# jaeyoungchoilab/Topsicle

Measured on AMD Instinct MI355X. Metric: bases_scanned_per_sec, higher is better.
Workload: dtype u8

## Files before the change

### __graft_entry__.py

```python
import os
import shutil
import subprocess
import sys

ROOT = os.path.dirname(os.path.abspath(__file__))
CSRC = os.path.join(ROOT, "topsicle_amd", "csrc")
LIB = os.path.join(ROOT, "topsicle_amd", "libtopsicle_hip.so")


def _newer(target, deps):
    return os.path.exists(target) and all(os.path.getmtime(target) >= os.path.getmtime(d) for d in deps)


HIP_FLAGS = ["--offload-arch=gfx950", "-O3", "-fno-vectorize", "-std=c++17", "-fPIC", "-Wall", "-Wno-unused-variable"]
KGROUPS = 18


def _build_hip_split(out, extra=()):
    hipcc = shutil.which("hipcc") or "/opt/rocm/bin/hipcc"
    flags = os.environ.get("TPS_HIPCC_EXTRA", "").split() + HIP_FLAGS + list(extra)
    bdir = os.path.join(CSRC, "_build", os.path.splitext(os.path.basename(out))[0])
    os.makedirs(bdir, exist_ok=True)
    jobs = []
    for g in range(KGROUPS):
        src = "topsicle_hip.hip" if g == 0 else "tps_kernels.hip"
        obj = os.path.join(bdir, f"group{g}.o")
        jobs.append((obj, subprocess.Popen([hipcc] + flags + [f"-DTPS_KGROUP={g}", "-c", "-o", obj, os.path.join(CSRC, src)], cwd=CSRC)))
    failed = [obj for obj, p in jobs if p.wait() != 0]
    if failed:
        raise RuntimeError("hipcc failed for " + ", ".join(failed))
    subprocess.check_call([hipcc, "--offload-arch=gfx950", "-shared", "-fPIC", "-o", out] + [obj for obj, _ in jobs], cwd=CSRC)
    return out


def build_hip(force=False):
    deps = [os.path.join(CSRC, f) for f in ("topsicle_hip.hip", "tps_kernels.hip", "tps_kernels.h", "tps_device.h", "tps_wave.h", "tps_plan.h", "tps_pack.h", "tps_wide.h", "tps_wide_plan.h", "tps_motif.h", "tps_variant.h", "tps_tract.h", "tps_ends.h", "tps_anchor.h", "tps_place.h", "tps_adapter.h", "tps_check.h", "tps_layout.h")] + \
           [os.path.join(ROOT, "include", "topsicle_hip.h")]
    if not force and _newer(LIB, deps):
        return LIB
    return _build_hip_split(LIB)


def build_hip_diag():
    return _build_hip_split(os.path.join(ROOT, "topsicle_amd", "libtopsicle_hip_diag.so"), extra=["-DTPS_STAMPS"])


def build_io(force=False):
    src = os.path.join(CSRC, "tps_io.cpp")
    out = os.path.join(ROOT, "topsicle_amd", "libtopsicle_io.so")
    if not force and _newer(out, [src, os.path.join(CSRC, "tps_pack.h"), os.path.join(CSRC, "tps_gzpar.h"), os.path.join(ROOT, "include", "topsicle_hip.h")]):
        return out
    subprocess.check_call(["g++", "-O2", "-std=c++17", "-shared", "-fPIC", "-Wall", "-o", out, src, "-lz", "-lpthread"])
    return out


def build_oracle():
    mk = os.path.join(ROOT, "oracle", "Makefile")
    if os.path.exists(mk):
        subprocess.check_call(["make", "-s", "-C", os.path.join(ROOT, "oracle")])


def build_emulation():
    sys.path.insert(0, os.path.join(ROOT, "tests"))
    sys.path.insert(0, ROOT)
    import emu_adapter_driver
    import emu_anchor_driver
    import emu_binseg_driver
    import emu_clear_driver
    import emu_driver
    import emu_ends_driver
    import emu_follow_wide_driver
    import emu_motif_driver
    import emu_place_driver
    import emu_tract_driver
    import emu_variant_driver
    import emu_wide_driver
    emu_driver.build()
    emu_binseg_driver.build()
    emu_wide_driver.build()
    emu_wide_driver.build_main()
    emu_follow_wide_driver.build()
    emu_motif_driver.build()
    emu_motif_driver.build_main()
    emu_variant_driver.build()
    emu_variant_driver.build_main()
    emu_tract_driver.build()
    emu_tract_driver.build_main()
    emu_ends_driver.build()
    emu_ends_driver.build_main()
    emu_anchor_driver.build()
    emu_anchor_driver.build_main()
    emu_place_driver.build()
    emu_place_driver.build_main()
    emu_adapter_driver.build()
    emu_adapter_driver.build_main()
    emu_clear_driver.build_main()
    import test_layout
    test_layout.build_main()


def build_sanitizer_variants():
    sys.path.insert(0, os.path.join(ROOT, "tests"))
    sys.path.insert(0, ROOT)
    import emu_driver
    import emu_follow_wide_driver
    import emu_wide_driver
    import test_sanitizers
    emu_driver.build(asan=True)
    emu_wide_driver.build(asan=True)
    emu_follow_wide_driver.build(asan=True)
    test_sanitizers._build_io_asan()


def build() -> None:
    import threading
    errs = []

    def side(fn):
        try:
            fn()
        except BaseException as e:
            errs.append(e)
    th = [threading.Thread(target=side, args=(fn,)) for fn in (build_emulation, build_sanitizer_variants)]
    for t in th:
        t.start()
    build_hip()
    build_io()
    build_oracle()
    for t in th:
        t.join()
    if errs:
        raise errs[0]
    sys.path.insert(0, ROOT)
    import topsicle_amd
    from topsicle_amd import hiplib
    lib = hiplib.load_library()
    assert lib.tps_abi_version() == 4
    print("built", LIB)


def _revcomp(s):
    return s[::-1].translate(str.maketrans("ACGT", "TGCA"))


def smoke() -> None:
    sys.path.insert(0, ROOT)
    sys.path.insert(0, os.path.join(ROOT, "oracle"))
    import numpy as np
    from topsicle_amd import hiplib, synth
    import topsicle_oracle as orc

    motif, k = "CCCTAA", 4
    pats = orc.kmer_table(motif, k)
    bases, offsets, _ = synth.make_reads(24, 3000, motif, seed=7, tract_min=300, tract_max=1500)
    seqs = synth.split_reads(bases, offsets)
    ratio = 1000 / len(motif)
    min_count = max(c for c in range(1001) if not (c / ratio > 0.4))
    with hiplib.HipScanner(0) as sc:
        print("smoke on:", sc.device_info())
        sc.set_patterns(pats)
        sc.upload(0, bases, offsets)
        prm = hiplib.make_params(min_len=1000, min_count=min_count, window=100, slide=6, trimfirst=100, maxlen=20000,
                                 flags=hiplib.F_STEP1 | hiplib.F_WINDOWS | hiplib.F_BINSEG | hiplib.F_STORE_SUMS)
        sc.scan(0, prm)
        sc.sync()
        res = sc.results(0)
        sums, win_off = sc.window_sums(0)
        sk, kept = sc.end_sketch(0, motif, res["tail"] != 0, [1500] * len(seqs), [3500] * len(seqs))
        degree, links, matches = sc.sketch_links(np.vstack([sk, sk]), 6, 4)
        assert (kept > 200).all() and (links[:len(seqs), 0] == np.arange(len(seqs)) + len(seqs)).all() and (matches[:len(seqs), 0] == (sk != 0xFFFFFFFF).sum(axis=1)).all()
        codes, keep = sc.end_window(0, motif, res["tail"] != 0, [1500] * len(seqs), [3500] * len(seqs))
        n_keep = np.array([sum(bin(int(x)).count("1") for x in row) for row in keep])
        offset, votes, second = sc.anchor_offsets(codes, keep, [1500] * len(seqs), list(range(len(seqs))), 2000)
        assert (n_keep == kept).all() and (offset == 0).all() and (2 * votes > kept).all() and (votes <= kept).all() and (4 * second < votes).all()
        p_ref, p_total, _, _, p_offset, p_votes, _ = sc.place_windows(codes, keep, [1500] * len(seqs), codes[:5], keep[:5], [1500] * 5, 2000)
        assert (p_ref[:5] == np.arange(5)).all() and (p_total[:5] >= kept[:5]).all() and (p_offset[:5] == 0).all() and (2 * p_votes[:5] > kept[:5]).all() and (p_votes[5:] < 20).all()
        ad = ["GATTACAGGCATCGTTCAGAGTCC", "TGCATCAGGTCCAAGTCAGGTTCA"]
        planted = seqs[0][:7] + ad[0][:11] + ad[0][12:] + seqs[0][30:] if res["tail"][0] == 0 else seqs[0][:-30] + _revcomp(ad[0][:11] + ad[0][12:]) + seqs[0][-7:]
        sc.upload(1, *hiplib.pack_reads([planted] + seqs[1:]))
        a_dist, a_end = sc.adapter_find(1, ad, res["tail"] != 0, [0] * len(seqs), [256] * len(seqs))
        assert (int(a_dist[0, 0]), int(a_end[0, 0])) == (1, 30) and (a_dist[1:, 0] > 5).all() and (a_dist[:, 1] > 5).all() and (a_end <= 256).all()
# ... 22 lines not shown
```

### include/topsicle_hip.h

```cpp
#ifndef TOPSICLE_HIP_H
#define TOPSICLE_HIP_H

#include <stdint.h>

#ifdef __cplusplus
extern "C" {
#endif

#define TPS_ABI_VERSION 4

#define TPS_OK            0
#define TPS_E_NO_DEVICE  -1
#define TPS_E_HIP        -2
#define TPS_E_ARG        -3
#define TPS_E_PATTERN    -4
#define TPS_E_CAPACITY   -5
#define TPS_E_STATE      -6

#define TPS_MAX_K         15
#define TPS_DIRECT_K      7
#define TPS_MAX_PATTERNS 31
#define TPS_WIDE_MAX_K        32
#define TPS_WIDE_MAX_PATTERNS 64

// ... 71 lines not shown
                               int64_t n_reads, int64_t n_words, int64_t* n_words_out);
int  tps_batch_set_tails(tps_ctx* ctx, int32_t slot, const uint8_t* tails);

int  tps_batch_scan(tps_ctx* ctx, int32_t slot, const tps_params* prm);
int  tps_sync(tps_ctx* ctx);
int  tps_batch_results(tps_ctx* ctx, int32_t slot, tps_read_result* out, int64_t n_reads);
int  tps_batch_window_offsets(tps_ctx* ctx, int32_t slot, int64_t* win_off, int64_t n_plus_1);
int  tps_batch_window_sums(tps_ctx* ctx, int32_t slot, int32_t* sums, int64_t n_windows);
int  tps_batch_window_raw(tps_ctx* ctx, int32_t slot, uint8_t* raw, int64_t n_windows_times_p);
typedef uint32_t (*tps_crc32_fn)(uint32_t crc, const uint8_t* p, int64_t n);
int  tps_batch_raw_to_fd(tps_ctx* ctx, int32_t slot, const int64_t* reads, int64_t n_sel, int fd, int64_t file_off,
                         tps_crc32_fn crc_fn, uint32_t* crc_out, int64_t* bytes_out);
int  tps_batch_read_sums(tps_ctx* ctx, int32_t slot, int64_t read, int32_t* sums, int64_t n_windows);
int  tps_batch_trc_counts(tps_ctx* ctx, int32_t slot, int32_t* c_start, int32_t* c_end, int64_t n_reads);

int  tps_trc_counts(tps_ctx* ctx, const uint8_t* bases, const int64_t* offsets, int64_t n_reads,
                    int32_t no_bp, int32_t* c_start, int32_t* c_end);
int  tps_window_counts(tps_ctx* ctx, const uint8_t* bases, const int64_t* offsets,
                       const uint8_t* tails, int64_t n_reads, int32_t window, int32_t slide,
                       int32_t trimfirst, int32_t maxlen, const int64_t* win_off,
                       int32_t* sums, uint8_t* raw);
int  tps_binseg_l2(tps_ctx* ctx, const int32_t* sums, const int64_t* win_off, int64_t n_reads,
                   int32_t n_patterns, int32_t jump, int32_t min_size, int32_t* bkp, double* gain);
int  tps_binseg_l2_ties(tps_ctx* ctx, const int32_t* sums, const int64_t* win_off, int64_t n_reads,
                        int32_t n_patterns, int32_t jump, int32_t min_size, int32_t* bkp, double* gain, uint8_t* tie);

int64_t tps_window_count(int64_t read_len, int32_t window, int32_t slide, int32_t trimfirst, int32_t maxlen);

int  tps_batch_kmer_followers(tps_ctx* ctx, int32_t slot, int32_t n_fwd, int32_t follow, int32_t lo, int32_t hi,
                              int32_t min_len, uint32_t* picks, int64_t picks_words, int64_t* hist, int64_t hist_len);
int  tps_batch_kmer_followers_wide(tps_ctx* ctx, int32_t slot, int32_t n_fwd, int32_t follow, int32_t lo, int32_t hi,
                                   int32_t min_len, uint32_t* picks, int64_t picks_words, int64_t* hist, int64_t hist_len);

typedef struct tps_motif_hit {
    uint64_t unit;
    int32_t period;
    int32_t support;
    int32_t run_start;
    int32_t run_len;
    int32_t n_bases;
    int32_t reserved;
} tps_motif_hit;
int  tps_batch_motif_census(tps_ctx* ctx, int32_t slot, int32_t u_min, int32_t u_max, int32_t lo, int32_t hi, int32_t min_len,
                            tps_motif_hit* hits, int64_t n_hits, int32_t* counts, int64_t counts_len);

int  tps_batch_variant_census(tps_ctx* ctx, int32_t slot, uint64_t unit, int32_t m, const uint8_t* tails, const int32_t* begin,
                              const int32_t* end, int64_t n_reads, int32_t bin, int32_t n_bins, uint32_t* counts,
                              int64_t counts_len, int64_t* profile, int64_t profile_len);

typedef struct tps_tract {
    int32_t begin, end;
    int32_t hits, blocks;
} tps_tract;
int  tps_batch_tract_map(tps_ctx* ctx, int32_t slot, uint64_t unit, int32_t m, int32_t block, int32_t min_hits, int32_t gap,
                         int32_t min_blocks, int32_t max_tracts, tps_tract* tracts, int64_t tracts_len, int32_t* found,
                         int64_t found_len, uint32_t* totals, int64_t totals_len);

int  tps_batch_end_sketch(tps_ctx* ctx, int32_t slot, uint64_t unit, int32_t m, int32_t k, int32_t buckets, const uint8_t* tails,
                          const int32_t* begin, const int32_t* end, int64_t n_reads, uint32_t* sketch, int64_t sketch_len,
                          uint32_t* kept, int64_t kept_len);
int  tps_sketch_links(tps_ctx* ctx, const uint32_t* sketch, int64_t n, int32_t buckets, int64_t sketch_len, int32_t min_match,
                      int32_t max_links, int32_t* degree, int64_t degree_len, int32_t* links, int64_t links_len, int32_t* matches,
                      int64_t matches_len);

int  tps_batch_end_window(tps_ctx* ctx, int32_t slot, uint64_t unit, int32_t m, int32_t k, const uint8_t* tails, const int32_t* begin,
                          const int32_t* end, int64_t n_reads, int32_t span, uint32_t* codes, int64_t codes_len, uint32_t* keep,
                          int64_t keep_len);
int  tps_window_offsets(tps_ctx* ctx, const uint32_t* codes, const uint32_t* keep, const int32_t* length, const int32_t* ref, int64_t n,
                        int32_t span, int32_t k, int32_t* offset, int32_t* votes, int32_t* second, int64_t out_len);

int  tps_window_place(tps_ctx* ctx, const uint32_t* codes, int64_t codes_len, const uint32_t* keep, int64_t keep_len, const int32_t* length,
                      int64_t n, const uint32_t* ref_codes, int64_t ref_codes_len, const uint32_t* ref_keep, int64_t ref_keep_len,
                      const int32_t* ref_length, int32_t n_ref, int32_t span, int32_t k, int32_t max_occ, int32_t* ref, int32_t* total,
                      int32_t* runner_ref, int32_t* runner, int32_t* offset, int32_t* votes, int32_t* second, int64_t out_len);

int  tps_batch_adapter_find(tps_ctx* ctx, int32_t slot, const uint64_t* patterns, const int32_t* pat_len, int32_t n_pat,
                            const uint8_t* tails, const int32_t* begin, const int32_t* end, int64_t n_reads, uint16_t* hits,
                            int64_t hits_len);

int  tps_kernel_time_ms(tps_ctx* ctx, int32_t* n_launches, double* total_ms, double* mean_ms);
int  tps_kernel_time_reset(tps_ctx* ctx);
int  tps_ctx_debug_option(tps_ctx* ctx, const char* key, int64_t value);
int  tps_debug_stamps_get(tps_ctx* ctx, int32_t slot, uint64_t* out, int64_t n_reads);
int  tps_device_info(tps_ctx* ctx, char* buf, int32_t buf_len);
int  tps_batch_kernel_info(tps_ctx* ctx, int32_t slot, char* buf, int32_t buf_len);

#ifdef __cplusplus
}
#endif
#endif
```

### topsicle_amd/csrc/topsicle_hip.hip

```cpp
#include <hip/hip_runtime.h>
#include <hip/hip_ext.h>

#include <sys/uio.h>
#include <unistd.h>

#include <algorithm>
#include <cerrno>
#include <cstdarg>
#include <cstdio>
#include <cstdlib>
#include <cstring>
#include <deque>
#include <initializer_list>
#include <map>
#include <mutex>
#include <set>
#include <string>
#include <vector>

#include "tps_device.h"
#include "tps_motif.h"
#include "tps_variant.h"
#include "tps_tract.h"
#include "tps_ends.h"
// ... 204 lines not shown
            uint64_t x;
            if (!rev) {
                x = nib_swap(q[w]);
            } else {
                const int64_t a = L - 16 - 16 * w;
                const int64_t qa = a >> 4;
                const uint32_t sh = (uint32_t)(a & 15) * 4u;
                const uint64_t lo = qa >= 0 ? nib_swap(q[qa]) : 0ull;
                x = sh ? (lo >> sh) | (nib_swap(q[qa + 1]) << (64u - sh)) : lo;
                x = __brevll(x);
            }
#pragma unroll
            for (int t = 0; t < 16; ++t) {
                const uint32_t c = (uint32_t)(x >> (4 * t)) & 15u;
                packed |= ((NIB4_CODE2 >> (2 * c)) & 3u) << (2 * t);
                bad |= ((~NIB4_ACGT >> c) & 1u) << t;
            }
            if (left < 16) {
                packed &= (1u << (2 * (int)left)) - 1u;
                bad &= (1u << (int)left) - 1u;
            }
        }
        seq2[w0 + w] = packed;
        inv[w0 + w] = (uint16_t)bad;
    }
}

namespace {

thread_local std::string g_err;

std::mutex g_pinned_mu;
std::map<uintptr_t, size_t> g_pinned;
bool is_pinned(const void* p, size_t bytes) {
    if (!p || !bytes) return true;
    std::lock_guard<std::mutex> lk(g_pinned_mu);
    auto it = g_pinned.upper_bound((uintptr_t)p);
    if (it == g_pinned.begin()) return false;
    --it;
    return (uintptr_t)p + bytes <= it->first + it->second;
}

int fail(int code, const char* fmt, ...) {
    char buf[512];
    va_list ap;
    va_start(ap, fmt);
    vsnprintf(buf, sizeof buf, fmt, ap);
    va_end(ap);
    g_err = buf;
    return code;
}

#define HIP_TRY(expr)                                                                        \
    do {                                                                                     \
        hipError_t e_ = (expr);                                                              \
        if (e_ != hipSuccess) return fail(TPS_E_HIP, "%s: %s", #expr, hipGetErrorString(e_)); \
    } while (0)

constexpr int64_t PAD = 64;
constexpr int INTERNAL_SLOT = TPS_MAX_SLOTS;

struct DevBuf {
    void* p = nullptr;
    size_t cap = 0;
    bool borrowed = false;
    DevBuf() = default;
    DevBuf(const DevBuf&) = delete;
    DevBuf& operator=(const DevBuf&) = delete;
    ~DevBuf() { release(); }
    int ensure(size_t bytes) {
        if (borrowed) { p = nullptr; cap = 0; borrowed = false; }
        if (bytes <= cap) return TPS_OK;
        if (p) { (void)hipFree(p); p = nullptr; cap = 0; }
        size_t want = bytes + bytes / 8 + 256;
        HIP_TRY(hipMalloc(&p, want));
        cap = want;
        return TPS_OK;
    }
    void release() { if (p && !borrowed) (void)hipFree(p); p = nullptr; cap = 0; borrowed = false; }
    void borrow(const DevBuf& o) { release(); p = o.p; cap = o.cap; borrowed = true; }
};

struct Slot {
    DevBuf seq2, inv, desc, tails, results, c_start, c_end, win_off, win_off16, sums, raw, stamps, lc, order;
    int64_t n_words = 0;
    bool inv_valid = true;
    bool any_invalid = true;
    std::vector<int64_t> h_offsets;
    tps::BatchLayout lay;
    std::vector<uint16_t> h_sums16;
    tps_read_result* h_results = nullptr;
    size_t h_results_cap = 0;
    int64_t n = -1;
    bool has_tails = false;
    bool planned = false;
    tps_params plan_prm{};
    int plan_k = 0, plan_p = 0;
    uint32_t plan_dup = 0, plan_so = 0;
    tps::ScanArgs args{};
    size_t lds_bytes = 0;
    const char* kernel_name = "";
    bool scanned = false;
    uint32_t last_flags = 0;
    Slot* sub = nullptr;
    bool sub_stale = true;
    void* ext_raw = nullptr;
    const int64_t* ext_raw_win_off = nullptr;
    bool rows_inline = false;
    int stride_base = 0;
    std::string info_name;
    bool wplanned = false;
    tps_params wplan_prm{};
    uint64_t wplan_table = 0;
    tps::WideArgs wargs{};
    ~Slot() {
        if (h_results) (void)hipHostFree(h_results);
        delete sub;
    }
};

struct ScanKernel { const void* fn; const char* name; };
#define TPS_K(sym) {(const void*)sym, #sym}
enum ScanFamily { KF_PLAIN, KF_PAIR, KF_PAIRQ, KF_RAW, KF_SO, KF_SOL, KF_SOR, KF_SORH, KF_COUNT };
constexpr int KSLIDE_MIN = 3, KSLIDE_MAX = 12;
const ScanKernel GENERIC_KERNEL = TPS_K(tps_scan_kernel);
const ScanKernel FUSED_KERNELS[KF_COUNT][KSLIDE_MAX - KSLIDE_MIN + 1] = {
    {TPS_K(tps_scan_kernel_s3), TPS_K(tps_scan_kernel_s4), TPS_K(tps_scan_kernel_s5), TPS_K(tps_scan_kernel_s6), TPS_K(tps_scan_kernel_s7),
     TPS_K(tps_scan_kernel_s8), TPS_K(tps_scan_kernel_s9), TPS_K(tps_scan_kernel_s10), TPS_K(tps_scan_kernel_s11), TPS_K(tps_scan_kernel_s12)},
    {TPS_K(tps_scan_kernel_s3p), TPS_K(tps_scan_kernel_s4p), TPS_K(tps_scan_kernel_s5p), TPS_K(tps_scan_kernel_s6p), TPS_K(tps_scan_kernel_s7p),
     TPS_K(tps_scan_kernel_s8p), TPS_K(tps_scan_kernel_s9p), TPS_K(tps_scan_kernel_s10p), TPS_K(tps_scan_kernel_s11p), TPS_K(tps_scan_kernel_s12p)},
    {{}, {}, TPS_K(tps_scan_kernel_s5q), TPS_K(tps_scan_kernel_s6q), TPS_K(tps_scan_kernel_s7q), TPS_K(tps_scan_kernel_s8q)},
    {{}, {}, TPS_K(tps_scan_kernel_s5r), TPS_K(tps_scan_kernel_s6r), TPS_K(tps_scan_kernel_s7r), TPS_K(tps_scan_kernel_s8r)},
    {{}, {}, TPS_K(tps_scan_kernel_s5so), TPS_K(tps_scan_kernel_s6so), TPS_K(tps_scan_kernel_s7so), TPS_K(tps_scan_kernel_s8so)},
    {{}, {}, TPS_K(tps_scan_kernel_s5sol), TPS_K(tps_scan_kernel_s6sol), TPS_K(tps_scan_kernel_s7sol), TPS_K(tps_scan_kernel_s8sol)},
    {{}, {}, TPS_K(tps_scan_kernel_s5sor), TPS_K(tps_scan_kernel_s6sor), TPS_K(tps_scan_kernel_s7sor), TPS_K(tps_scan_kernel_s8sor)},
    {{}, {}, TPS_K(tps_scan_kernel_s5sorh), TPS_K(tps_scan_kernel_s6sorh), TPS_K(tps_scan_kernel_s7sorh), TPS_K(tps_scan_kernel_s8sorh)},
};
#undef TPS_K

struct EventPair { hipEvent_t a, b; };

}

struct tps_ctx {
    int device = 0;
    hipStream_t stream = nullptr;
    hipDeviceProp_t prop{};
    struct Table { DevBuf dev; int P = 0, k = 0; std::string key; tps::PatInfo pat{}; size_t off_e32 = 0, off_fld = 0, off_m16 = 0, off_f16 = 0, off_p16 = 0, off_pfld = 0; };
    std::deque<Table> tables;
    Table* lut_cur = nullptr;
    struct WideTable { DevBuf dev; std::string key; int P = 0, k = 0; tps::WidePat pat{}; uint64_t serial = 0; };
    std::deque<WideTable> wtables;
    WideTable* wide_cur = nullptr;
    size_t wtable_rr = 0;
    uint64_t table_serial = 0;
    size_t lds_set_wide = 0;
    size_t table_rr = 0;
    DevBuf follow_picks, follow_hist;
    DevBuf motif_hits, motif_counts;
    DevBuf variant_in, variant_counts, variant_prof;
    std::vector<unsigned long long> h_variant_prof;
    DevBuf tract_table, tract_out;
    DevBuf ends_in, ends_out;
    DevBuf links_t, links_out;
    DevBuf window_out;
    DevBuf offsets_in, offsets_out;
    DevBuf place_in, place_idx, place_out;
    DevBuf adapter_in, adapter_out;
    DevBuf ascii, ascii_off;
    DevBuf nib, nib_src;
    std::set<void*> pinned;
    std::vector<tps_read_desc> h_desc;
    tps::PatInfo pat{};
// ... 335 lines not shown
        sl.wplan_table = wt.serial;
        sl.wplanned = true;
    }
    sl.planned = false;
    sl.args = tps::ScanArgs{};
    sl.args.wpg = sl.wargs.wpg;
    sl.plan_p = P;
    sl.plan_k = wt.k;
    sl.stride_base = 0;
    sl.rows_inline = false;
    sl.lds_bytes = (size_t)tps::wide_wg_lds_dwords(sl.wargs) * 4;
    static const char wide_name[] = "tps_scan_kernel_wide";
    sl.kernel_name = wide_name;
    sl.last_flags = prm.flags;
    const int64_t total_win = sl.lay.win_off[(size_t)n];
    if ((rc = ensure_h_results(sl, n))) return rc;
    tps::WideArgs& a = sl.wargs;
    a.seq2 = (const uint32_t*)sl.seq2.p;
    a.inv = (const uint16_t*)sl.inv.p;
    a.desc = (const tps_read_desc*)sl.desc.p;
    a.tails_in = ((prm.flags & TPS_F_TAILS_IN) && !(prm.flags & TPS_F_STEP1)) ? (const uint8_t*)sl.tails.p : nullptr;
    a.img = (const uint32_t*)wt.dev.p;
    a.results = sl.h_results;
    a.c_start = a.c_end = nullptr;
    if (prm.flags & TPS_F_STEP1) {
        if ((rc = sl.c_start.ensure((size_t)std::max<int64_t>(n * P, 1) * 4))) return rc;
        if ((rc = sl.c_end.ensure((size_t)std::max<int64_t>(n * P, 1) * 4))) return rc;
        a.c_start = (int32_t*)sl.c_start.p;
        a.c_end = (int32_t*)sl.c_end.p;
    }
    a.win_off = (const int64_t*)sl.win_off.p;
    a.order = sl.lay.order.empty() ? nullptr : (const int32_t*)sl.order.p;
    a.sums = nullptr;
    a.raw = nullptr;
    if (prm.flags & TPS_F_WINDOWS) {
        if ((rc = sl.sums.ensure((size_t)std::max<int64_t>(total_win, 1) * 4))) return rc;
        a.sums = (int32_t*)sl.sums.p;
    }
    if (prm.flags & TPS_F_STORE_RAW) {
        if ((rc = sl.raw.ensure((size_t)std::max<int64_t>(total_win * P, 1)))) return rc;
        a.raw = (uint8_t*)sl.raw.p;
    }
    a.n_reads = n;
    a.prm = prm;
    if (n == 0) { sl.scanned = true; return TPS_OK; }
    if (c->poison) {
        if ((rc = poison_h_results(c, sl))) return rc;
        if (a.c_start) { TPS_POISON(sl.c_start); TPS_POISON(sl.c_end); }
        if (a.sums) TPS_POISON(sl.sums);
        if (a.raw) TPS_POISON(sl.raw);
    }
    if (sl.lds_bytes > c->lds_set_wide) {
        HIP_TRY(hipFuncSetAttribute((const void*)tps_scan_kernel_wide, hipFuncAttributeMaxDynamicSharedMemorySize, (int)sl.lds_bytes));
        c->lds_set_wide = sl.lds_bytes;
    }
    EventPair ev;
    if ((rc = next_events(c, false, ev))) return rc;
    const int64_t grid = (n + a.wpg - 1) / a.wpg;
    void* kargs[] = {(void*)&a};
    HIP_TRY(hipExtLaunchKernel((const void*)tps_scan_kernel_wide, dim3((unsigned)grid), dim3(tps::NT * a.wpg), kargs, sl.lds_bytes, c->stream,
                               ev.a, ev.b, 0));
    sl.scanned = true;
    return TPS_OK;
}

int do_scan(tps_ctx* c, Slot& sl, const tps_params& prm, bool inner, hipEvent_t ev_start) {
    int rc;
    if (!c->have_pat) return fail(TPS_E_PATTERN, "tps_set_patterns has not been called");
    if ((rc = check_scan(sl, prm))) return rc;
    if (c->wide_cur) return do_scan_wide(c, sl, prm);
    const int64_t n = sl.n;
    const int P = c->pat.P;
    if (!sl.planned || !same_params(prm, sl.plan_prm) || sl.plan_k != c->pat.k || sl.plan_p != P ||
        (sl.plan_dup != 0) != (c->pat.dup_mask != 0) || (sl.plan_so != 0) != (c->pat.so_mask != 0)) {
        tps::plan_batch_layout(sl.h_offsets.data(), n, prm, sl.lay);
        if (c->file_order) sl.lay.order.clear();
        if (!sl.lay.order.empty()) {
            if ((rc = sl.order.ensure((size_t)n * 4))) return rc;
            HIP_TRY(hipMemcpyAsync(sl.order.p, sl.lay.order.data(), (size_t)n * 4, hipMemcpyHostToDevice, c->stream));
        }
        sl.args = tps::ScanArgs{};
        sl.args.val_on = sl.any_invalid ? 1 : 0;
        if ((rc = plan_lds(c, sl, prm, sl.lay.max_nwin))) return rc;
        sl.stride_base = 0;
        if (!inner && !c->no_stride) {
            sl.stride_base = tps::stride_base(sl.args, prm, c->pat.k, P, [&](int s0) { return window_count(sl.lay.max_len, prm.window, s0, prm.trimfirst, prm.maxlen); },
                                              lds_budget_dw(c), c->knobs);
        }
        if ((rc = sl.win_off.ensure((size_t)(n + 1) * 8))) return rc;
        HIP_TRY(hipMemcpyAsync(sl.win_off.p, sl.lay.win_off.data(), (size_t)(n + 1) * 8, hipMemcpyHostToDevice, c->stream));
        if (sl.args.variant) {
            if ((rc = sl.win_off16.ensure((size_t)(n + 1) * 8))) return rc;
            HIP_TRY(hipMemcpyAsync(sl.win_off16.p, sl.lay.win_off16.data(), (size_t)(n + 1) * 8, hipMemcpyHostToDevice, c->stream));
        }
        HIP_TRY(hipStreamSynchronize(c->stream));
        sl.plan_prm = prm;
        sl.plan_k = c->pat.k;
        sl.plan_p = P;
        sl.plan_dup = c->pat.dup_mask;
        sl.plan_so = c->pat.so_mask;
        sl.planned = true;
    }
    const int64_t total_win = sl.lay.win_off[(size_t)n];
    if ((rc = ensure_h_results(sl, n))) return rc;
    tps::ScanArgs& a = sl.args;
    a.seq2 = (const uint32_t*)sl.seq2.p;
    a.inv = (const uint16_t*)sl.inv.p;
    a.desc = (const tps_read_desc*)sl.desc.p;
    a.tails_in = ((prm.flags & TPS_F_TAILS_IN) && !(prm.flags & TPS_F_STEP1)) ? (const uint8_t*)sl.tails.p : nullptr;
    a.lut = (const uint32_t*)c->lut_cur->dev.p;
    a.pair_img = a.lut + (a.pair16 ? c->lut_cur->off_p16 : (a.lut_fields && a.pair_n) ? c->lut_cur->off_pfld : (size_t)a.lut_n);
    a.lut_img = a.lut + ((a.lut16 && a.lut_fields) ? c->lut_cur->off_f16 : a.lut16 ? c->lut_cur->off_m16 : a.lut_fields ? c->lut_cur->off_fld : c->lut_cur->off_e32);
    a.results = sl.h_results;
    if (inner) {
        if ((rc = sl.results.ensure((size_t)std::max<int64_t>(n, 1) * sizeof(tps_read_result)))) return rc;
        a.results = (tps_read_result*)sl.results.p;
    }
    a.c_start = a.c_end = nullptr;
    if ((prm.flags & TPS_F_STEP1) && !sl.stride_base) {
        if ((rc = sl.c_start.ensure((size_t)std::max<int64_t>(n * P, 1) * 4))) return rc;
        if ((rc = sl.c_end.ensure((size_t)std::max<int64_t>(n * P, 1) * 4))) return rc;
        a.c_start = (int32_t*)sl.c_start.p;
        a.c_end = (int32_t*)sl.c_end.p;
    }
    a.win_off = (const int64_t*)sl.win_off.p;
    a.order = sl.lay.order.empty() ? nullptr : (const int32_t*)sl.order.p;
    a.sums = nullptr;
    a.sums16 = nullptr;
    a.win_off16 = nullptr;
    a.raw = nullptr;
    if (prm.flags & TPS_F_WINDOWS) {
        if (a.variant) {
            if ((rc = sl.sums.ensure((size_t)std::max<int64_t>(sl.lay.win_off16[(size_t)n], 8) * 2))) return rc;
            a.sums16 = (uint16_t*)sl.sums.p;
            a.win_off16 = (const int64_t*)sl.win_off16.p;
        } else {
            if ((rc = sl.sums.ensure((size_t)std::max<int64_t>(total_win, 1) * 4))) return rc;
            a.sums = (int32_t*)sl.sums.p;
        }
    }
    a.raw_m = 0;
    a.raw_win_off = nullptr;
    sl.rows_inline = false;
    if (prm.flags & TPS_F_STORE_RAW) {
        if (inner && sl.ext_raw && a.variant && a.pp_d >= 0 && (c->pat.so_mask == 0 ? a.pp_d == 0 : a.pp_d > 0) && (P & 3) == 0 && !sl.any_invalid) {
            a.raw = (uint8_t*)sl.ext_raw;
            a.raw_m = 2;
            a.raw_win_off = sl.ext_raw_win_off;
            sl.rows_inline = true;
        } else {
            if ((rc = sl.raw.ensure((size_t)std::max<int64_t>(total_win * P, 1)))) return rc;
            a.raw = (uint8_t*)sl.raw.p;
        }
    }
    a.lc_scratch = nullptr;
    if (a.lc_global) {
        if ((rc = sl.lc.ensure((size_t)std::max<int64_t>(n, 1) * (size_t)a.lc_stride * 2))) return rc;
        a.lc_scratch = (uint16_t*)sl.lc.p;
    }
    if (c->poison) {
        if (inner) TPS_POISON(sl.results);
        else if ((rc = poison_h_results(c, sl))) return rc;
        if (a.c_start) { TPS_POISON(sl.c_start); TPS_POISON(sl.c_end); }
        if (a.sums || a.sums16) TPS_POISON(sl.sums);
        if (a.raw && !sl.rows_inline) TPS_POISON(sl.raw);
        if (a.lc_scratch) TPS_POISON(sl.lc);
    }
    a.stamps = nullptr;
    if (c->want_stamps) {
        if ((rc = sl.stamps.ensure((size_t)std::max<int64_t>(n, 1) * 16 * 8))) return rc;
        TPS_POISON(sl.stamps);
        HIP_TRY(hipMemsetAsync(sl.stamps.p, 0, (size_t)std::max<int64_t>(n, 1) * 16 * 8, c->stream));
        a.stamps = (uint64_t*)sl.stamps.p;
    }
    a.n_reads = n;
    a.pat = c->pat;
    a.prm = prm;
    sl.last_flags = prm.flags;
    if (n == 0) { sl.scanned = true; return TPS_OK; }

    const ScanKernel* k = &GENERIC_KERNEL;
    size_t* lds_set = &c->lds_set_generic;
    if (tps::has_specialised_slide(a.variant) || tps::has_default_only_slide(a.variant)) {
        const ScanFamily fam = scan_family(a, a.raw != nullptr);
        k = &FUSED_KERNELS[fam][a.variant - KSLIDE_MIN];
        lds_set = &c->lds_set_fused[fam][a.variant - KSLIDE_MIN];
    }
    sl.kernel_name = k->name;
    if (sl.lds_bytes > *lds_set) {
        HIP_TRY(hipFuncSetAttribute(k->fn, hipFuncAttributeMaxDynamicSharedMemorySize, (int)sl.lds_bytes));
        *lds_set = sl.lds_bytes;
    }
    EventPair ev;
    if ((rc = next_events(c, inner, ev))) return rc;
    if (sl.stride_base) {
        if ((rc = do_scan_strided(c, sl, prm, sl.stride_base, ev.a, ev.b))) return rc;
        sl.scanned = true;
        return TPS_OK;
    }
    {
        const int64_t grid = (n + a.wpg - 1) / a.wpg;
        void* kargs[] = {(void*)&a};
        HIP_TRY(hipExtLaunchKernel(k->fn, dim3((unsigned)grid), dim3(tps::NT * a.wpg), kargs, sl.lds_bytes, c->stream,
                                   inner ? ev_start : ev.a, ev.b, 0));
    }
    sl.scanned = true;
    return TPS_OK;
}

Slot* get_slot(tps_ctx* c, int slot) {
    if (!c || slot < 0 || slot >= TPS_MAX_SLOTS) { fail(TPS_E_ARG, "slot out of range"); return nullptr; }
    return &c->slots[slot];
}


int need_slot(tps_ctx* c, int slot, Slot** out) {
    int rc;
    if ((rc = bind(c))) return rc;
    return (*out = get_slot(c, slot)) ? TPS_OK : TPS_E_ARG;
}
int have_batch(const Slot& sl) { return sl.n < 0 ? fail(TPS_E_STATE, "no batch uploaded in this slot") : TPS_OK; }
int need_batch(tps_ctx* c, int slot, Slot** out) {
    int rc;
    if ((rc = need_slot(c, slot, out))) return rc;
    return have_batch(**out);
}

template <class A>
void set_batch(A& a, const Slot& sl) {
    a.seq2 = (const uint32_t*)sl.seq2.p;
    a.inv = (const uint16_t*)sl.inv.p;
    a.desc = (const tps_read_desc*)sl.desc.p;
}

template <class T>
T* at(const DevBuf& b, size_t off) { return (T*)((char*)b.p + off); }

template <class A>
int upload_region(tps_ctx* c, const DevBuf& buf, const tps::RegionAt& r, const uint8_t* tails, const int32_t* begin, const int32_t* end, int64_t n, A& a) {
    a.tails = at<const uint8_t>(buf, r.tails);
    a.begin = at<const int32_t>(buf, r.begin);
    a.end = at<const int32_t>(buf, r.end);
    HIP_TRY(hipMemcpyAsync((void*)a.tails, tails, (size_t)n, hipMemcpyHostToDevice, c->stream));
    HIP_TRY(hipMemcpyAsync((void*)a.begin, begin, (size_t)n * 4, hipMemcpyHostToDevice, c->stream));
    HIP_TRY(hipMemcpyAsync((void*)a.end, end, (size_t)n * 4, hipMemcpyHostToDevice, c->stream));
    return TPS_OK;
}
// ... 654 lines not shown
    const tps::RegionAt reg = tps::region_layout(in, n);
    if ((rc = c->adapter_in.ensure(in.total))) return rc;
    if ((rc = c->adapter_out.ensure(out_bytes))) return rc;
    TPS_POISON(c->adapter_out);
    tps::AdapterArgs a{};
    set_batch(a, *sl);
    a.peq = at<const uint64_t>(c->adapter_in, off_peq);
    a.pat_len = at<const int32_t>(c->adapter_in, off_len);
    HIP_TRY(hipMemcpyAsync((void*)a.peq, peq, peq_bytes, hipMemcpyHostToDevice, c->stream));
    HIP_TRY(hipMemcpyAsync((void*)a.pat_len, pat_len, len_bytes, hipMemcpyHostToDevice, c->stream));
    if ((rc = upload_region(c, c->adapter_in, reg, tails, begin, end, n, a))) return rc;
    a.hits = (uint32_t*)c->adapter_out.p;
    a.n_reads = n;
    a.n_pat = n_pat;
    if ((rc = launch_waves(c, tps::adapter_find_kernel, n, tps::ADAPTER_WPG, a))) return rc;
    return download(c, {{hits, a.hits, out_bytes}});
}

int tps_batch_set_tails(tps_ctx* c, int32_t slot, const uint8_t* tails) {
    int rc;
    if ((rc = bind(c))) return rc;
    Slot* sl = get_slot(c, slot);
    if (!sl) return TPS_E_ARG;
    if (sl->n < 0) return fail(TPS_E_STATE, "no batch uploaded in this slot");
    if (!tails && sl->n > 0) return fail(TPS_E_ARG, "null tails");
    if ((rc = sl->tails.ensure((size_t)std::max<int64_t>(sl->n, 1)))) return rc;
    if (sl->n) HIP_TRY(hipMemcpyAsync(sl->tails.p, tails, (size_t)sl->n, hipMemcpyHostToDevice, c->stream));
    HIP_TRY(hipStreamSynchronize(c->stream));
    sl->has_tails = true;
    return TPS_OK;
}

int tps_batch_scan(tps_ctx* c, int32_t slot, const tps_params* prm) {
    int rc;
    if ((rc = bind(c))) return rc;
    Slot* sl = get_slot(c, slot);
    if (!sl) return TPS_E_ARG;
    if (!prm) return fail(TPS_E_ARG, "null params");
    return do_scan(c, *sl, *prm);
}

int tps_sync(tps_ctx* c) {
    int rc;
    if ((rc = bind(c))) return rc;
    HIP_TRY(hipStreamSynchronize(c->stream));
    return TPS_OK;
}

static int need_scanned(tps_ctx* c, int slot, Slot** out) {
    int rc;
    if ((rc = bind(c))) return rc;
    Slot* sl = (slot == INTERNAL_SLOT) ? &c->slots[INTERNAL_SLOT] : get_slot(c, slot);
    if (!sl) return TPS_E_ARG;
    if (!sl->scanned) return fail(TPS_E_STATE, "slot has not been scanned");
    HIP_TRY(hipStreamSynchronize(c->stream));
    *out = sl;
    return TPS_OK;
}

int tps_batch_results(tps_ctx* c, int32_t slot, tps_read_result* out, int64_t n) {
    Slot* sl;
    int rc;
    if ((rc = need_scanned(c, slot, &sl))) return rc;
    if (n != sl->n || (n > 0 && !out)) return fail(TPS_E_ARG, "result buffer must hold %lld reads", (long long)sl->n);
    if (n) memcpy(out, sl->h_results, (size_t)n * sizeof(tps_read_result));
    return TPS_OK;
}

int tps_batch_window_offsets(tps_ctx* c, int32_t slot, int64_t* win_off, int64_t n1) {
    Slot* sl;
    int rc;
    if ((rc = need_scanned(c, slot, &sl))) return rc;
    if (n1 != sl->n + 1 || !win_off) return fail(TPS_E_ARG, "win_off must hold n+1 entries");
    memcpy(win_off, sl->lay.win_off.data(), (size_t)n1 * 8);
    return TPS_OK;
}

int tps_batch_window_sums(tps_ctx* c, int32_t slot, int32_t* sums, int64_t nw) {
    Slot* sl;
    int rc;
    if ((rc = need_scanned(c, slot, &sl))) return rc;
    if (!(sl->last_flags & TPS_F_STORE_SUMS)) return fail(TPS_E_STATE, "last scan did not store window sums");
    if (nw != sl->lay.win_off[(size_t)sl->n] || (nw > 0 && !sums)) return fail(TPS_E_ARG, "sums must hold %lld windows", (long long)sl->lay.win_off[(size_t)sl->n]);
    if (nw && sl->args.variant) {
        const int64_t n16 = sl->lay.win_off16[(size_t)sl->n];
        sl->h_sums16.resize((size_t)n16);
        HIP_TRY(hipMemcpy(sl->h_sums16.data(), sl->sums.p, (size_t)n16 * 2, hipMemcpyDeviceToHost));
        tps::widen_sums16(sl->h_sums16.data(), sl->lay.win_off16.data(), sl->lay.win_off.data(), 0, sl->n, sums);
    } else if (nw) {
        HIP_TRY(hipMemcpy(sums, sl->sums.p, (size_t)nw * 4, hipMemcpyDeviceToHost));
    }
    tps::clear_skipped_windows(sl->h_results, sl->lay.win_off.data(), sl->n, 1, 4, 0, nw, sums);
    return TPS_OK;
}

int tps_batch_read_sums(tps_ctx* c, int32_t slot, int64_t read, int32_t* sums, int64_t nw) {
    Slot* sl;
    int rc;
    if ((rc = need_scanned(c, slot, &sl))) return rc;
    if (!(sl->last_flags & TPS_F_WINDOWS)) return fail(TPS_E_STATE, "last scan did not run the window step");
    if (read < 0 || read >= sl->n) return fail(TPS_E_ARG, "read %lld out of range", (long long)read);
    const int64_t lo = sl->lay.win_off[(size_t)read], cnt = sl->lay.win_off[(size_t)read + 1] - lo;
    if (nw != cnt || (nw > 0 && !sums)) return fail(TPS_E_ARG, "sums must hold %lld windows", (long long)cnt);
    if (!nw) return TPS_OK;
    if (sl->args.variant) {
        sl->h_sums16.resize((size_t)nw);
        HIP_TRY(hipMemcpy(sl->h_sums16.data(), (const uint16_t*)sl->sums.p + sl->lay.win_off16[(size_t)read], (size_t)nw * 2, hipMemcpyDeviceToHost));
        for (int64_t w = 0; w < nw; ++w) sums[w] = (int32_t)sl->h_sums16[(size_t)w];
    } else {
        HIP_TRY(hipMemcpy(sums, (const int32_t*)sl->sums.p + lo, (size_t)nw * 4, hipMemcpyDeviceToHost));
    }
    tps::clear_skipped_windows(sl->h_results, sl->lay.win_off.data(), sl->n, 1, 4, lo, lo + nw, sums);
    return TPS_OK;
}

int tps_batch_window_raw(tps_ctx* c, int32_t slot, uint8_t* raw, int64_t nwp) {
    Slot* sl;
    int rc;
    if ((rc = need_scanned(c, slot, &sl))) return rc;
    if (!(sl->last_flags & TPS_F_STORE_RAW)) return fail(TPS_E_STATE, "last scan did not store raw counts");
    int64_t want = sl->lay.win_off[(size_t)sl->n] * sl->plan_p;
    if (nwp != want || (nwp > 0 && !raw)) return fail(TPS_E_ARG, "raw must hold %lld bytes", (long long)want);
    if (nwp) HIP_TRY(hipMemcpy(raw, sl->raw.p, (size_t)nwp, hipMemcpyDeviceToHost));
    tps::clear_skipped_windows(sl->h_results, sl->lay.win_off.data(), sl->n, sl->plan_p, 1, 0, nwp, raw);
    return TPS_OK;
}

constexpr size_t RAW_STAGE = (size_t)32 << 20;
constexpr int64_t RAW_GAP = 256 << 10;

int tps_batch_raw_to_fd(tps_ctx* c, int32_t slot, const int64_t* reads, int64_t n_sel, int fd, int64_t file_off,
                        tps_crc32_fn crc_fn, uint32_t* crc_out, int64_t* bytes_out) {
    Slot* sl;
    int rc;
    if ((rc = need_scanned(c, slot, &sl))) return rc;
    if (!(sl->last_flags & TPS_F_STORE_RAW)) return fail(TPS_E_STATE, "last scan did not store raw counts");
    if (n_sel < 0 || (n_sel > 0 && !reads) || fd < 0 || file_off < 0) return fail(TPS_E_ARG, "bad arguments");
    if (crc_out) *crc_out = 0;
    if (bytes_out) *bytes_out = 0;
    const int64_t P = sl->plan_p;
    struct Run { int64_t lo, hi; };
    std::vector<Run> runs;
    int64_t prev = -1;
    for (int64_t j = 0; j < n_sel; ++j) {
        const int64_t i = reads[j];
        if (i <= prev || i >= sl->n) return fail(TPS_E_ARG, "reads[] must be ascending indices of the batch (entry %lld)", (long long)j);
        prev = i;
        const int64_t lo = sl->lay.win_off[(size_t)i] * P, hi = sl->lay.win_off[(size_t)i + 1] * P;
        if (hi == lo) continue;
        if (!runs.empty() && runs.back().hi == lo) runs.back().hi = hi;
        else runs.push_back({lo, hi});
    }
    if (runs.empty()) return TPS_OK;
    for (int i = 0; i < 2; ++i) {
        if (!c->raw_stage[i]) HIP_TRY(hipHostMalloc(&c->raw_stage[i], RAW_STAGE, hipHostMallocPortable));
        if (!c->raw_ev[i]) HIP_TRY(hipEventCreateWithFlags(&c->raw_ev[i], hipEventDisableTiming));
    }
    struct Piece { size_t r0, r1; int64_t lo, hi; };
    std::vector<Piece> pieces;
    {
        std::vector<Run> cut;
        size_t i = 0;
        int64_t pos = runs[0].lo;
        while (i < runs.size()) {
            Piece pc{cut.size(), cut.size(), pos, pos};
            while (i < runs.size()) {
                const int64_t start = std::max(pos, runs[i].lo);
                if (pc.r1 > pc.r0 && (start - pc.hi > RAW_GAP || start >= pc.lo + (int64_t)RAW_STAGE)) break;
                if (pc.r1 == pc.r0) pc.lo = start;
                const int64_t end = std::min(runs[i].hi, pc.lo + (int64_t)RAW_STAGE);
                if (end <= start) break;
                cut.push_back({start, end});
                pc.r1 = cut.size();
                pc.hi = end;
                pos = end;
                if (end == runs[i].hi) { ++i; if (i < runs.size()) pos = runs[i].lo; }
                else break;
            }
            pieces.push_back(pc);
        }
        runs.swap(cut);
    }
    auto enqueue = [&](size_t j) -> int {
        const Piece& pc = pieces[j];
        HIP_TRY(hipMemcpyAsync(c->raw_stage[j & 1], (const uint8_t*)sl->raw.p + pc.lo, (size_t)(pc.hi - pc.lo), hipMemcpyDeviceToHost, c->stream));
        HIP_TRY(hipEventRecord(c->raw_ev[j & 1], c->stream));
        return TPS_OK;
    };
// ... 105 lines not shown
    if (nw > 0 && !sums) return fail(TPS_E_ARG, "null sums");
    for (int64_t i = 0; i < n; ++i) {
        const int64_t lo = win_off[i], len = win_off[i + 1] - lo;
        if (len < 0 || lo < 0 || lo + len > nw) return fail(TPS_E_ARG, "win_off not monotone at %lld", (long long)i);
        if (len > 500000) return fail(TPS_E_CAPACITY, "read %lld has %lld windows (max 500000)", (long long)i, (long long)len);
        uint64_t tot = 0;
        for (int64_t w = 0; w < len; ++w) {
            if (sums[lo + w] < 0) return fail(TPS_E_ARG, "negative window sum at read %lld", (long long)i);
            tot += (uint64_t)sums[lo + w];
        }
        if (tot >> 32 || (double)len * (double)len * (double)tot >= 18446744073709551616.0)
            return fail(TPS_E_CAPACITY, "window sums of read %lld exceed the change-point arithmetic (total %llu over %lld windows)",
                        (long long)i, (unsigned long long)tot, (long long)len);
    }
    Slot& sl = c->slots[INTERNAL_SLOT];
    if ((rc = sl.sums.ensure((size_t)std::max<int64_t>(nw, 1) * 4))) return rc;
    if ((rc = sl.win_off.ensure((size_t)(n + 1) * 8))) return rc;
    if ((rc = sl.results.ensure((size_t)n * 17))) return rc;
    TPS_POISON(sl.results);
    sl.planned = false;
    sl.wplanned = false;
    sl.scanned = false;
    if (nw) HIP_TRY(hipMemcpyAsync(sl.sums.p, sums, (size_t)nw * 4, hipMemcpyHostToDevice, c->stream));
    HIP_TRY(hipMemcpyAsync(sl.win_off.p, win_off, (size_t)(n + 1) * 8, hipMemcpyHostToDevice, c->stream));
    tps::BinsegArgs a{};
    a.sums = (const int32_t*)sl.sums.p;
    a.win_off = (const int64_t*)sl.win_off.p;
    a.gain = (double*)sl.results.p;
    a.bkp = (int32_t*)((char*)sl.results.p + (size_t)n * 8);
    a.tie = (uint8_t*)sl.results.p + (size_t)n * 12;
    a.n_reads = n;
    a.n_patterns = n_patterns;
    a.jump = jump;
    a.min_size = min_size;
    hipLaunchKernelGGL(tps_binseg_kernel, dim3((unsigned)((n + tps::WPG - 1) / tps::WPG)), dim3(tps::NT * tps::WPG), 0, c->stream, a);
    HIP_TRY(hipGetLastError());
    HIP_TRY(hipMemcpyAsync(bkp, a.bkp, (size_t)n * 4, hipMemcpyDeviceToHost, c->stream));
    if (gain) HIP_TRY(hipMemcpyAsync(gain, a.gain, (size_t)n * 8, hipMemcpyDeviceToHost, c->stream));
    if (tie) HIP_TRY(hipMemcpyAsync(tie, a.tie, (size_t)n, hipMemcpyDeviceToHost, c->stream));
    HIP_TRY(hipStreamSynchronize(c->stream));
    return TPS_OK;
}

int tps_kernel_time_ms(tps_ctx* c, int32_t* n_launches, double* total_ms, double* mean_ms) {
    int rc;
    if ((rc = bind(c))) return rc;
    HIP_TRY(hipStreamSynchronize(c->stream));
    double tot = 0.0;
    for (size_t i = c->ev_base; i < c->ev_used; ++i) {
        float ms = 0.f;
        HIP_TRY(hipEventElapsedTime(&ms, c->ev_pool[i].a, c->ev_pool[i].b));
        tot += ms;
    }
    const size_t cnt = c->ev_used - c->ev_base;
    if (n_launches) *n_launches = (int32_t)cnt;
    if (total_ms) *total_ms = tot;
    if (mean_ms) *mean_ms = cnt ? tot / (double)cnt : 0.0;
    return TPS_OK;
}

int tps_ctx_debug_option(tps_ctx* c, const char* key, int64_t value) {
    if (!c || !key) return fail(TPS_E_ARG, "null argument");
    const std::string k(key);
    if (k == "event_stride") c->event_stride = (int)std::max<int64_t>(1, value);
    else if (k == "no_events") c->no_events = value != 0;
    else if (k == "force_generic") c->knobs.force_generic = value != 0;
    else if (k == "spans_per_tile") c->knobs.spans_per_tile = (int)std::max<int64_t>(0, value);
    else if (k == "force_pair") c->knobs.force_pair = value != 0;
    else if (k == "so_order") c->knobs.so_order = (int)value;
    else if (k == "wpg") c->knobs.wpg = (int)value;
    else if (k == "stamps") c->want_stamps = value != 0;
    else if (k == "file_order") c->file_order = value != 0;
    else if (k == "no_stride") c->no_stride = value != 0;
    else if (k == "no_inline_rows") c->no_inline_rows = value != 0;
    else if (k == "poison") {
        if (value < 0 || value > 255) return fail(TPS_E_ARG, "poison must be 0 (off) or a fill byte 1..255");
        c->poison = (int)value;
    }
    else return fail(TPS_E_ARG, "unknown debug option '%s' (event_stride, no_events, force_generic, spans_per_tile, force_pair, so_order, wpg, stamps, file_order, no_stride, no_inline_rows, poison)", key);
    drop_plans(c);
    return TPS_OK;
}

int tps_debug_stamps_get(tps_ctx* c, int32_t slot, uint64_t* out, int64_t n) {
    Slot* sl;
    int rc;
    if ((rc = need_scanned(c, slot, &sl))) return rc;
    if (!sl->stamps.p || n != sl->n) return fail(TPS_E_STATE, "no stamps recorded");
    HIP_TRY(hipMemcpy(out, sl->stamps.p, (size_t)n * 16 * 8, hipMemcpyDeviceToHost));
    return TPS_OK;
}

int tps_kernel_time_reset(tps_ctx* c) {
    int rc;
    if ((rc = bind(c))) return rc;
    HIP_TRY(hipStreamSynchronize(c->stream));
    c->ev_base = c->ev_used;
    c->launch_seq = 0;
    return TPS_OK;
}

}
```

### topsicle_amd/csrc/tps_device.h

```cpp
#pragma once
#include <stdint.h>
#include "../../include/topsicle_hip.h"
#include "tps_wave.h"
#include "tps_check.h"

namespace tps {

constexpr int WPG = 4;
constexpr int WPG_MAX = 8;
constexpr uint32_t FLAG_CONFLICT = 0x80000000u;
constexpr uint32_t FLAG16 = 0x8000u;
constexpr int HIST_COPIES = 8;
constexpr int WIN_U = 4;
constexpr int COOP_MAX = 24;

typedef unsigned __int128 u128;

constexpr int cgcd(int a, int b) { return b == 0 ? a : cgcd(b, a % b); }
constexpr int clog2(int x) { return x <= 1 ? 0 : 1 + clog2(x / 2); }

struct PatInfo {
    int32_t P, k;
    uint32_t kmask;
    uint32_t all_mask;
    uint32_t so_mask;
    uint32_t dup_mask;
    int32_t n_periods;
    int32_t period[8];
    uint32_t period_pat[8];
    uint32_t hash_mul, hash_shift;
};

struct ScanArgs {
    const uint32_t* seq2;
    const uint16_t* inv;
    const tps_read_desc* desc;
    const uint8_t* tails_in;
    const uint32_t* lut;
    const uint32_t* lut_img;
    const uint32_t* pair_img;
    tps_read_result* results;
    int32_t* c_start;
    int32_t* c_end;
    const int64_t* win_off;
    int32_t* sums;
    uint16_t* sums16;
    const int64_t* win_off16;
    uint8_t* raw;
    uint64_t* stamps;
    int32_t raw_m;
    const int64_t* raw_win_off;
    const int32_t* order;
    int64_t n_reads;
    PatInfo pat;
    tps_params prm;
    int32_t variant;
    int32_t lut_n;
    int32_t seq_dw;
    int32_t head_dw;
    int32_t nblk_cap;
    int32_t spans_per_tile;
    int32_t span_dw;
    int32_t blk_log2;
    int32_t rec_rs;
    int32_t tot_dw;
    int32_t blk_dw;
    int32_t lc_cap;
    uint32_t jump_magic;
    int32_t q, r, lw;
    int32_t lc_global;
    int32_t lc_stride;
    uint16_t* lc_scratch;
    int32_t pair_n;
    int32_t tw;
    int32_t tile_full;
    int32_t wpg;
    int32_t pp_d;
    int32_t so_fast;
    int32_t val_on;
    int32_t seq_alias;
    int32_t lut_fields;
    int32_t lut16;
    int32_t xt_alias;
    int32_t xt_own;
    int32_t pair16;
};

struct BinsegArgs {
    const int32_t* sums;
    const int64_t* win_off;
    int32_t* bkp;
    double* gain;
    int64_t n_reads;
    int32_t n_patterns, jump, min_size;
    uint8_t* tie;
};

constexpr int MISC_DW = 20;
constexpr int XS_DW = 64 + NT + 4 * NT + NT + 16 * 5 + 8;
constexpr int HIST_STRIDE = 33;
constexpr int HIST_DW = 2 * HIST_COPIES * HIST_STRIDE;
struct Lds {
    uint32_t* lut;
    uint32_t* lut2;
    int lshift;
    uint32_t* seq2;
    uint16_t* val;
    uint32_t* blk;
    uint32_t* G;
    uint32_t* Gp;
    uint16_t* C0;
    uint16_t* C1;
    uint32_t* XPC;
    uint32_t* XF;
    uint32_t* XT;
    uint32_t* Tot;
    uint32_t* row;
    uint32_t* misc;
};
constexpr int XLANES = NT + 16;
TPS_HD int64_t xchg_dw(const ScanArgs& a) {
    return 9ll * NT + (a.xt_alias == 2 ? 0ll : 2ll) * XLANES;
}
TPS_HD int64_t lut_dw(const ScanArgs& a) { return a.lut16 ? ((((int64_t)a.lut_n + 1) / 2 + 3) & ~3ll) : (((int64_t)a.lut_n + 3) & ~3ll); }
TPS_HD int64_t blk_region_dw(const ScanArgs& a) {
    int64_t need = a.variant ? xchg_dw(a) : 2ll * a.nblk_cap + 2ll * ((a.nblk_cap + 1) / 2);
    if (need < XS_DW) need = XS_DW;
    if (need < HIST_DW) need = HIST_DW;
    return (need + 3) & ~3ll;
}
TPS_HD int64_t val_dw(const ScanArgs& a) { return a.val_on ? ((a.seq_dw + 4 + 3) / 4) * 2 : 0; }
TPS_HD int64_t row_dw(const ScanArgs& a) {
    const int64_t fused = a.variant ? ((int64_t)NT << a.blk_log2) + NT : 0;
    return fused > WIN_U * NT ? fused : WIN_U * NT;
}
TPS_DEV Lds carve(uint32_t* base, uint32_t* lut, const ScanArgs& a) {
    Lds l;
    l.lut2 = lut - a.pair_n;
    uint32_t* p = base;
    l.blk = p;  p += a.blk_dw;
    l.lut = lut;
    l.lshift = a.variant ? 16 : 0;
    l.seq2 = p; p += a.seq_dw;
    l.val = (uint16_t*)p;  p += val_dw(a);
    l.Tot = p;  p += a.tot_dw;
    l.row = p;  p += row_dw(a);
    l.misc = p;
    l.G = l.blk;
    l.Gp = l.G + a.nblk_cap;
    l.C0 = (uint16_t*)(l.Gp + a.nblk_cap);
    l.C1 = l.C0 + ((a.nblk_cap + 1) / 2) * 2;
    l.XPC = l.blk;
    l.XF = l.XPC + 9 * NT;
    l.XT = l.XF + XLANES;
    return l;
}
TPS_HD int64_t lds_dwords(const ScanArgs& a) {
    return (int64_t)a.blk_dw + (a.seq_alias ? 0 : a.seq_dw) + val_dw(a) + a.tot_dw + row_dw(a) + MISC_DW +
           ((a.xt_alias && a.xt_own) ? (a.xt_alias == 2 ? 2 : 1) * XLANES : 0);
}
TPS_HD int64_t wg_lds_dwords(const ScanArgs& a) { return a.pair_n + lut_dw(a) + (int64_t)(a.wpg > 0 ? a.wpg : WPG) * ((lds_dwords(a) + 3) & ~3ll); }
constexpr int M_BEST = 0;
constexpr int M_CMASK = 2;
constexpr int M_INVALID = 4;
constexpr int M_SCAN = 10;
constexpr int M_MAXSC = 6;
constexpr int M_BESTB = 8;
constexpr int M_NTIE = 9;
// ... 666 lines not shown
            scan_positions(l, pat, q0, a.lw, inv, [&](int p, uint32_t h) {
                if ((h >> bit) & 1u) {
                    ++occ;
                    if (p >= cursor) { ++greedy; cursor = p + pat.k; }
                }
            });
            sum -= (uint32_t)(occ - greedy);
        }
        return sum;
    }
    uint64_t clo = 0, chi = 0, c3 = 0, c4 = 0;
    scan_positions(l, pat, q0, a.lw, inv, [&](int, uint32_t h) {
        while (h) {
            const int b = ffs0(h);
            h &= h - 1;
            const uint64_t inc = 1ull << (8 * (b & 7));
            const int g = b >> 3;
            clo += g == 0 ? inc : 0ull;
            chi += g == 1 ? inc : 0ull;
            c3 += g == 2 ? inc : 0ull;
            c4 += g == 3 ? inc : 0ull;
        }
    });
    uint32_t sum = 0;
    for (int b = 0; b < pat.P; ++b) {
        const uint64_t word = (b >> 3) == 0 ? clo : (b >> 3) == 1 ? chi : (b >> 3) == 2 ? c3 : c4;
        int c = (int)((word >> (8 * (b & 7))) & 255u);
        if ((redo >> b) & 1u) {
            int greedy = 0, cursor = 0;
            scan_positions(l, pat, q0, a.lw, inv, [&](int p, uint32_t h) {
                if (((h >> b) & 1u) && p >= cursor) { ++greedy; cursor = p + pat.k; }
            });
            c = greedy;
        }
        if (c == 0) c = 1;
        if (raw_row) raw_row[b] = (uint8_t)c;
        sum += (uint32_t)c;
    }
    return sum;
}

TPS_DEV void windows_group(const ScanArgs& a, const Lds& l, int delta, int w0, int nw_tile, int64_t out_base, int base, int tid) {
    const PatInfo& pat = a.pat;
    const int q = a.q;
    for (int u = 0; u < WIN_U; ++u) {
        const int wl = base + u * NT + tid;
        uint32_t sw = 0;
        if (wl < nw_tile) {
            uint32_t m = l.Gp[wl + q];
            for (int i = 0; i < q; ++i) m |= l.G[wl + i];
            int je = wl + q;
            uint32_t cnt = ((uint32_t)l.C1[je] + l.Tot[je >> a.blk_log2]) - ((uint32_t)l.C0[wl] + l.Tot[wl >> a.blk_log2]);
            uint32_t present = m & pat.all_mask;
            sw = cnt + (uint32_t)(pat.P - popc(present));
            uint8_t* raw_row = a.raw ? a.raw + (out_base + w0 + wl) * (int64_t)pat.P : nullptr;
            if ((m & FLAG_CONFLICT) || raw_row) sw = window_exact(a, l, delta, wl, present, sw, raw_row);
            a.sums[out_base + w0 + wl] = (int32_t)sw;
        }
        l.row[u * NT + tid] = sw;
    }
}

TPS_DEV uint32_t div_jump(uint32_t w, uint32_t magic) { return magic ? (uint32_t)(((uint64_t)w * magic) >> 32) : w; }
TPS_DEV void candidates_group(const ScanArgs& a, const Lds& l, uint64_t lc_g, int w0, int nw_tile, int base, uint32_t carry, int tid) {
    const uint32_t jump = (uint32_t)a.prm.jump;
    TPS_UNROLL
    for (int u = 0; u < WIN_U; ++u) {
        const int wl = base + u * NT + tid;
        if (wl < nw_tile) {
            const uint32_t w = (uint32_t)(w0 + wl);
            const uint32_t c = div_jump(w, a.jump_magic);
            if (c * jump == w && (int)c < a.lc_cap) {
                g32_store(lc_g, c, carry + l.row[u * NT + tid]);
            }
        }
    }
}

struct TileConst {
    int32_t q, r;
    uint32_t jump, jump_magic, lc_cap;
    uint64_t lc_g;
    uint16_t* sw16;
    int64_t rd;
};
TPS_DEV TileConst tile_const(const ScanArgs& a, int64_t r) {
    TileConst t;
    t.lc_g = (uint64_t)(uintptr_t)(a.lc_scratch + r * (int64_t)a.lc_stride);
    t.sw16 = a.sums16 + (a.win_off16 ? a.win_off16[r] : 0);
    t.rd = r;
    t.q = (int32_t)uniform((uint32_t)a.q); t.r = (int32_t)uniform((uint32_t)a.r);
    t.jump = uniform((uint32_t)a.prm.jump); t.jump_magic = uniform(a.jump_magic);
    t.lc_cap = uniform((uint32_t)a.lc_cap);
    TPS_PIN_S(t.q); TPS_PIN_S(t.r); TPS_PIN_S(t.jump); TPS_PIN_S(t.jump_magic); TPS_PIN_S(t.lc_cap);
    return t;
}

template <int S>
struct Geo {
    static constexpr int B = 8;
    static constexpr int LOG2B = 3;
    static constexpr int C = 8;
    static constexpr int LOG2C = 3;
    static constexpr int POS = B * S;
    static constexpr int WDW = (POS + 13 + 15) / 16;
};
constexpr int SEQ_LEAD = 4;
template <int S, bool FULL>
struct TileGeo {
    static constexpr int LANES = FULL ? NT : NT - 1;
    static constexpr int BASES = LANES * Geo<S>::POS + 13 + 15;
    static constexpr int NQ = (63 + BASES + 63) / 64;
    static constexpr int PF = (NQ + NT - 1) / NT;
    static constexpr int SEQ_TILE = SEQ_LEAD + 4 * NQ + 4;
    static constexpr int SEQ = SEQ_TILE < 144 ? 144 : SEQ_TILE;
};
constexpr bool tile_full_default(int s) { return s >= 1; }

template <int S, bool FULL>
TPS_DEV Lds carve_fused(uint32_t* base, uint32_t* lut, const ScanArgs& a) {
    constexpr int BLK = 9 * NT, ROW = NT * Geo<S>::B + NT, SEQ = TileGeo<S, FULL>::SEQ;
    const int VAL = a.val_on ? ((SEQ + 4 + 3) / 4) * 2 : 0;
    static_assert(BLK % 4 == 0 && ROW % 4 == 0 && MISC_DW % 4 == 0 && SEQ % 4 == 0, "seq2 must be 16-byte aligned");
    static_assert(BLK + ROW - SEQ >= HIST_DW && BLK + ROW - SEQ >= 4 * NT, "step 1 counts in front of the aliased bases");
    Lds l;
    l.lut2 = lut - a.pair_n;
    l.lut = lut;
    l.lshift = (a.lut16 && !a.lut_fields && !a.pair16) ? LUT_M16 : (a.lut_fields && a.lut16) ? LUT_F16 : a.lut_fields ? LUT_FIELDS : 16;
    l.blk = base;
    l.XPC = base;
    l.G = l.Gp = base; l.C0 = l.C1 = (uint16_t*)base;
    l.row = base + BLK;
    l.misc = l.row + ROW;
    l.Tot = l.misc + MISC_DW;
    uint32_t* p = l.Tot + 4;
    if (a.seq_alias) {
        l.seq2 = base + (BLK + ROW - SEQ);
    } else {
        l.seq2 = p;
        p += SEQ;
    }
    l.val = (uint16_t*)p;
    p += VAL;
    l.XF = p;
    l.XT = l.XF + XLANES;
    return l;
}

TPS_DEV uint32_t pack_hi_lo(uint32_t hi_src, uint32_t lo_src) { return perm(hi_src, lo_src, 0x07060100u); }

template <int S, bool SO, bool INV, int RPT, bool RAW>
TPS_DEV void tile_fused_s(const ScanArgs& a, const TileConst& tc, const Lds& l, int delta, int w0, int tile, int nw_tile,
                          int64_t out_base, uint64_t& s_total, int64_t r) {
    constexpr bool RZ = RPT == 0;
    typedef Geo<S> g_;
    constexpr int WDW = g_::WDW, B = g_::B, LOG2B = g_::LOG2B, POS = g_::POS;
    constexpr int RS = NT + NT / B;
    const PatInfo& pat = a.pat;
    const int rp = RPT >= 0 ? RPT : tc.r, q = tc.q;
    const uint32_t amask = pat.kmask << 2;
    TPS_PHASE {
        const int span = tid;
        const int p0 = delta + span * POS;
        const uint32_t sh2 = (uint32_t)((p0 - 1) & 15) * 2u;
        const int d0 = (p0 - 1) >> 4;
        uint32_t w[WDW];
        {
            uint32_t prev = l.seq2[d0];
            TPS_UNROLL
            for (int i = 0; i < WDW; ++i) {
                uint32_t nx = l.seq2[d0 + i + 1];
                w[i] = alignbit(nx, prev, sh2);
// ... 604 lines not shown
        uint32_t* const sw = TPS_AT(sw_);
        uint32_t* const swp = TPS_AT(swp_);
        const uint32_t* const sfx = TPS_AT(sfx_);
        const uint32_t* const c0s = TPS_AT(c0s_);
        const uint32_t* pe = l.XPC + (lane + dl0) * (B + 1) + rot;
        uint32_t ev[B];
        TPS_UNROLL
        for (int j = 0; j < B; ++j) ev[j] = pe[j + ((!ROTZ && j >= brk) ? 1 : 0)];
        uint32_t orw = 0, sumw = TPS_AT(xf_own);
        TPS_NOVEC
        for (int t = 1; t < dl0; ++t) {
            const uint32_t v = xf_at(lane + t);
            orw |= v;
            sumw += v;
        }
        uint32_t orb = orw, sumb = sumw;
        if (!ROTZ) {
            const uint32_t vb = xf_at(lane + dl0);
            orb |= vb;
            sumb += vb;
        }
        const uint32_t am = pat.all_mask << 16;
        orw |= ~am;
        orb |= ~am;
        uint32_t run = 0;
        if constexpr (SWP) {
            if (tid == 0) TPS_EMU_COUNT(3);
            uint32_t lo_lo = 0x05040100u;
            TPS_PIN_S(lo_lo);
            TPS_UNROLL
            for (int j = 0; j < B; j += 2) {
                const uint32_t ep = perm(ev[j + 1], ev[j], lo_lo), cp = perm(c0s[j + 1], c0s[j], lo_lo);
                const uint32_t d = pk_u16_add(pk_u16_sub(ep, cp), sumw);
                const uint32_t p = (uint32_t)popc(~(sfx[j] | ev[j] | orw)) + d;
                swp[j >> 1] = p + ((uint32_t)popc(~(sfx[j + 1] | ev[j + 1] | orw)) << 16);
                sw[j] = swp[j >> 1] & 0xFFFFu;
                sw[j + 1] = swp[j >> 1] >> 16;
                run += sw[j] + sw[j + 1];
            }
        } else {
        TPS_UNROLL
        for (int j = 0; j < B; ++j) {
            const bool far_ = !ROTZ && j >= brk;
            const uint32_t e = ev[j], fo = far_ ? orb : orw, fs = far_ ? sumb : sumw;
            const uint32_t c = (e - c0s[j] + fs) & 0xFFFFu;
            sw[j] = (CD > 0 ? (c & 0xFFu) - (c >> 8) : c) + (uint32_t)popc(~(sfx[j] | e | fo));
            run += sw[j];
        }
        }
        TPS_AT(ltot) = run;
    }
    TPS_ISA_MARK(MK + 3);
    if constexpr (CD > 0) {
        const bool tile_chain = lane_chain != 0;
        if (tile_chain) {
            TPS_EMU_COUNT(5);
            LaneArr<uint32_t, B> pd;
            Lane<uint32_t> dt(0);
            TPS_PHASE {
                const uint32_t* pr = l.row + tid * (B + 1);
                TPS_UNROLL
                for (int j = 0; j < B; ++j) { TPS_AT(dt) += pr[j]; TPS_AT(pd)[j] = TPS_AT(dt); }
            }
            const Lane<uint32_t> dbase = wave_excl_sum(dt);
            TPS_LANES {
                uint32_t run = 0;
                TPS_UNROLL
                for (int j = 0; j < B; ++j) { TPS_AT(sw_)[j] += TPS_AT(dbase) + TPS_AT(pd)[j]; run += TPS_AT(sw_)[j]; }
                TPS_AT(ltot) = run;
            }
        } else {
            TPS_EMU_COUNT(6);
        }
    }
    const Lane<uint32_t> lexc = wave_excl_sum(ltot);
    bool lane_cands = false;
    if constexpr (CD == 0 && !M16) lane_cands = tc.jump >= 4u;
    const uint32_t c_lo = div_jump((uint32_t)w0 + tc.jump - 1u, tc.jump_magic);
    uint32_t c_hi = div_jump((uint32_t)(w0 + nw_tile) + tc.jump - 1u, tc.jump_magic);
    if (c_hi > tc.lc_cap) c_hi = tc.lc_cap;
    TPS_PHASE {
        const int lane = tid;
        const uint32_t* const sw = TPS_AT(sw_);
        if constexpr (SWP) g_store_sw8p(tc.sw16 + w0, lane, nw_tile, TPS_AT(swp_));
        else g_store_sw8(tc.sw16 + w0, lane, nw_tile, sw);
        uint32_t* pr = l.row + lane * (B + 1);
        uint32_t run = 0;
        TPS_UNROLL
        for (int j = 0; j < B; ++j) { pr[j] = run; run += sw[j]; }
        xt_at(lane) = TPS_AT(lexc);
        if (lane_cands) {
            if (tid == 0) TPS_EMU_COUNT(7);
            auto own_candidates = [&](auto bigj_) {
                const uint32_t carry = (uint32_t)s_total + TPS_AT(lexc);
                const uint32_t wa = (uint32_t)w0 + (uint32_t)(lane * B);
                const uint32_t c = mulhi32(wa + tc.jump - 1u, tc.jump_magic);
                const uint32_t f = c * tc.jump - wa, f2 = f + tc.jump;
                uint32_t i1 = c, r1 = f;
                if constexpr (decltype(bigj_)::value != 0) {
                    i1 = f < (uint32_t)B ? c : c_hi;
                    r1 = f < (uint32_t)B ? f : (uint32_t)(B - 1);
                }
                const uint32_t i2 = (f2 < (uint32_t)B ? c : c_hi) + 1u;
                const uint32_t r2 = f2 < (uint32_t)B ? f2 : (uint32_t)(B - 1);
                const uint32_t v1 = pr[r1], v2 = pr[r2];
                g32_store_clamped(tc.lc_g, c_hi, i1, carry + v1);
                g32_store_clamped(tc.lc_g, c_hi, i2, carry + v2);
            };
            if (tc.jump > (uint32_t)B) own_candidates(IntC<1>());
            else own_candidates(IntC<0>());
        }
    }
    TPS_SYNC();
    if (w0 == 0) TPS_STAMP(12);
    TPS_ISA_MARK(MK + 4);
    const uint32_t gsum = uniform(l.row[nw_tile + (nw_tile >> LOG2B)] + xt_at(nw_tile >> LOG2B));
    {
        const uint32_t jump = tc.jump;
        const int passes = (c_hi > c_lo && !lane_cands) ? (int)((c_hi - c_lo + NT - 1) / NT) : 0;
        TPS_ISA_MARK(MK + 6);
        TPS_PHASE {
            const uint32_t carry = (uint32_t)s_total;
            if (tid == 0) { l.misc[M_INVALID] = 0; l.misc[M_NTIE] = 0; }
            uint32_t c = c_lo + (uint32_t)tid;
            uint32_t w = c * jump - (uint32_t)w0;
            TPS_NOVEC
            for (int t = 0; t < passes; ++t) {
                if (c < c_hi) {
                    const uint32_t pre = l.row[w + (w >> LOG2B)] + xt_at((int)(w >> LOG2B));
                    g32_store(tc.lc_g, c, carry + pre);
                }
                c += NT;
                w += NT * jump;
            }
        }
    }
    s_total += gsum;
    TPS_ISA_MARK(MK + 5);
    TPS_SYNC();
    (void)r;
}

template <int S>
struct GeoPP {
    static constexpr int B = 8, POS = B * S, LBK = 16;
    static constexpr int WDW = (1 + LBK + POS + 6 + 7 + 15) / 16;
};
constexpr uint32_t PP_BIAS = 14;
TPS_DEV void pp_expand(uint32_t ne, uint32_t no, uint32_t* b) {
    b[0] = ne & 0x0F0F0F0Fu;
    b[1] = (ne >> 4) & 0x0F0F0F0Fu;
    b[2] = no & 0x0F0F0F0Fu;
    b[3] = (no >> 4) & 0x0F0F0F0Fu;
}

template <int S, int D, int CD = 0, bool F16 = false, int RPT = -1, bool PAIRF = false>
TPS_DEV bool tile_pp_s(const ScanArgs& a, const TileConst& tc, const Lds& l, int delta, int w0, int tile, int nw_tile,
                       int64_t out_base, uint64_t& s_total) {
    static_assert(CD == 0 || (D == 0 && CD <= 6), "chain detection runs on the tile without self-overlap logic");
    static_assert(RPT < S, "r is a position inside a block");
    static_assert(!PAIRF || (D == 0 && CD == 0 && !F16 && RPT >= 0 && (RPT & 1) == 0), "pair lookups: plain tiles, the partial block ends between two pairs");
    constexpr int B = 8, POS = B * S, LBK = D > 0 ? 2 * D + 2 : 0;
    constexpr int WDW = (1 + LBK + POS + 6 + 7 + 15) / 16;
    constexpr int DH = D > 0 ? D : 1;
    constexpr int AHEAD = (D > 0 && 2 * D > S) ? 2 * D - S : 0;
    constexpr uint32_t M3 = 0x33333333u;
    const PatInfo& pat = a.pat;
// ... 388 lines not shown
        for (int j = 0; j < B; ++j) l.row[tid * (B + 1) + j] = TPS_AT(swv_)[j];
        if constexpr (CD > 0) {
            if (tid == clane) {
                TPS_UNROLL
                for (int i = 0; i < 7; ++i) carry[i] = 0u;
            }
        }
    }
    TPS_SYNC();
    if (D > 0) {
        TPS_FENCE_WG();
        TPS_PHASE {
            const int lane = tid;
            uint32_t todo = TPS_AT(todo_);
            const uint32_t chw = TPS_AT(chw_);
            while (todo) {
                const int bit = ffs0(todo);
                todo &= todo - 1u;
                const int j = bit & 7, wl = lane * B + j;
                if (wl >= nw_tile) continue;
                uint8_t* raw_row = a.raw ? a.raw + (out_base + w0 + wl) * (int64_t)pat.P : nullptr;
                if (a.raw && a.raw_m == 2)
                    raw_row = ((w0 + wl) & 1) ? nullptr : a.raw + (a.raw_win_off[tc.rd] + ((w0 + wl) >> 1)) * (int64_t)pat.P;
                uint32_t sw = l.row[lane * (B + 1) + j];
                if (bit < 8) {
                    TPS_EMU_COUNT(1);
                    sw = window_exact(a, l, delta, wl, pat.all_mask, 0u, raw_row, true);
                } else {
                    TPS_EMU_COUNT(3);
                    const int a0 = delta + wl * S;
                    uint32_t fw = chw;
                    bool lost = false;
                    while (fw) {
                        const int fidx = ffs0(fw) >> 1, pidx = pp_pattern(fidx);
                        fw &= fw - 1u;
                        int x = -1;
                        TPS_NOVEC
                        for (int i = 0; i < D; ++i)
                            if ((lut_mask(l.lut, l.lshift, pat, v_at(l.seq2, a0 + i)) >> pidx) & 1u) x = a0 + i;
                        if (x >= 0) {
                            int n = 0, pb = x - D;
                            while (pb >= delta && ((lut_mask(l.lut, l.lshift, pat, v_at(l.seq2, pb)) >> pidx) & 1u)) { ++n; pb -= D; }
                            const bool blocked = pb < delta && picked_before_tile(pb, fidx);
                            if (pb < delta && w0 != 0 && cold[6]) lost = true;
                            int m = 1;
                            for (int pw = x + D; pw < a0 + a.lw && ((lut_mask(l.lut, l.lshift, pat, v_at(l.seq2, pw)) >> pidx) & 1u); pw += D) ++m;
                            if ((((n & 1) != 0) != blocked) && (m & 1) == 0) {
                                sw -= 1u;
                                if (raw_row) raw_row[pidx] = (uint8_t)(raw_row[pidx] - 1u);
                            }
                        }
                    }
                    if (lost) {
                        TPS_EMU_COUNT(1);
                        sw = window_exact(a, l, delta, wl, pat.all_mask, 0u, raw_row, true);
                    }
                }
                l.row[lane * (B + 1) + j] = sw;
                tc.sw16[w0 + wl] = (uint16_t)sw;
            }
        }
        TPS_SYNC();
    }
    TPS_PP_STAMP(11);
    tile_candidates(tc, l, w0, tile, nw_tile, s_total);
    TPS_PP_STAMP(12);
    return false;
}

struct Cand { uint64_t d; uint64_t den; int32_t b; };
TPS_DEV bool cand_better(const Cand& x, const Cand& y) {
    if (x.b < 0) return false;
    if (y.b < 0) return true;
    u128 lhs = (u128)x.d * x.d * y.den;
    u128 rhs = (u128)y.d * y.d * x.den;
    if (lhs != rhs) return lhs > rhs;
    return x.b > y.b;
}
TPS_DEV bool binseg_admissible(int n, int jump, int min_size) {
    if (n / jump < 1) return false;
    int need = ((min_size + jump - 1) / jump) * jump + min_size;
    return need <= n;
}
template <typename ST>
TPS_DEV Cand binseg_chunk(const ST* S, int n, int jump, int min_size, int lo, int hi, uint64_t prefix, uint64_t total) {
    Cand best{0, 1, -1};
    uint64_t run = prefix;
    for (int b = lo; b < hi; ++b) {
        if (b % jump == 0 && b >= min_size && n - b >= min_size) {
            int64_t d = (int64_t)n * (int64_t)run - (int64_t)total * (int64_t)b;
            Cand c{(uint64_t)(d < 0 ? -d : d), (uint64_t)b * (uint64_t)(n - b), b};
            if (cand_better(c, best)) best = c;
        }
        run += (uint64_t)S[b];
    }
    return best;
}
TPS_DEV double score_f64(int64_t d, uint64_t den) {
    double x = (double)d;
    return x * x / (double)den;
}
TPS_DEV double gain_from(int64_t d, uint64_t den, int n, int n_patterns) {
    double x = (double)d;
    return x * x / ((double)n * (double)den) / ((double)n_patterns * (double)n_patterns);
}

template <typename ST>
TPS_DEV Cand binseg_exact_wg(const ST* S, int n, int jump, int min_size, uint32_t* xs) {
    const int cl = (n + NT - 1) / NT;
    TPS_PHASE {
        int lo = tid * cl, hi = lo + cl < n ? lo + cl : n;
        uint32_t sm = 0;
        for (int i = lo; i < hi; ++i) sm += (uint32_t)S[i];
        xs[X_BS + tid] = sm;
    }
    TPS_SYNC();
    constexpr int NG = NT / 16;
    TPS_PHASE {
        if (tid < NG) {
            uint32_t sm = 0;
            for (int i = 0; i < 16; ++i) sm += xs[X_BS + tid * 16 + i];
            xs[X_Q + tid] = sm;
        }
    }
    TPS_SYNC();
    TPS_PHASE {
        if (tid == 0) {
            uint32_t run = 0;
            for (int i = 0; i < NG; ++i) { uint32_t t = xs[X_Q + i]; xs[X_Q + i] = run; run += t; }
            xs[X_Q + 16] = run;
        }
    }
    TPS_SYNC();
    TPS_PHASE {
        uint64_t pre = xs[X_Q + (tid >> 4)];
        for (int i = (tid & ~15); i < tid; ++i) pre += xs[X_BS + i];
        int lo = tid * cl, hi = lo + cl < n ? lo + cl : n;
        Cand c = binseg_chunk(S, n, jump, min_size, lo, hi, pre, (uint64_t)xs[X_Q + 16]);
        ((uint64_t*)&xs[X_CD])[tid] = c.d;
        ((uint64_t*)&xs[X_CDEN])[tid] = c.den;
        ((int32_t*)&xs[X_CB])[tid] = c.b;
    }
    TPS_SYNC();
    TPS_PHASE {
        if (tid < NG) {
            Cand best{0, 1, -1};
            for (int i = 0; i < 16; ++i) {
                int t = tid * 16 + i;
                Cand c{((uint64_t*)&xs[X_CD])[t], ((uint64_t*)&xs[X_CDEN])[t], ((int32_t*)&xs[X_CB])[t]};
                if (cand_better(c, best)) best = c;
            }
            ((uint64_t*)&xs[X_R])[tid] = best.d;
            ((uint64_t*)&xs[X_R + 32])[tid] = best.den;
            ((int32_t*)&xs[X_R + 64])[tid] = best.b;
        }
    }
    TPS_SYNC();
    Cand best{0, 1, -1};
    for (int i = 0; i < NG; ++i) {
        Cand c{((uint64_t*)&xs[X_R])[i], ((uint64_t*)&xs[X_R + 32])[i], ((int32_t*)&xs[X_R + 64])[i]};
        if (cand_better(c, best)) best = c;
    }
    TPS_SYNC();
    return best;
}

constexpr int CHUNK_REGS = 16;
template <typename ST>
TPS_DEV void binseg_wg(const ST* S, int n, int jump, int min_size, int n_patterns, uint32_t* bs, uint32_t* misc,
                       uint32_t* xs, int& bkp, double& gain, bool& tie) {
    const int per = (n + jump * NT - 1) / (jump * NT);
    const int cl = per * jump;
    const bool in_regs = cl <= CHUNK_REGS;
    TPS_PHASE {
        const int lo = tid * cl, hi = lo + cl < n ? lo + cl : n;
        uint32_t sm = 0;
        if (in_regs) {
            TPS_UNROLL
            for (int i = 0; i < CHUNK_REGS; ++i)
                if (lo + i < hi) sm += (uint32_t)S[lo + i];
        } else {
            for (int i = lo; i < hi; ++i) sm += (uint32_t)S[i];
        }
        bs[tid] = sm;
        if (tid == 0) { *(uint64_t*)&misc[M_MAXSC] = 0ull; misc[M_BESTB] = (uint32_t)-1; misc[M_NTIE] = 0u; }
    }
    TPS_SYNC();
    const uint64_t tot = wg_exclusive_scan(bs, NT, &misc[M_SCAN]);
    Lane<double> best_(-1.0), second_(-1.0);
    Lane<int> best_b_(-1);
    TPS_PHASE {
        double &best = TPS_AT(best_), &second = TPS_AT(second_);
        int& best_b = TPS_AT(best_b_);
        const int lo = tid * cl, hi = lo + cl < n ? lo + cl : n;
        uint64_t run = bs[tid];
        best = -1.0; second = -1.0; best_b = -1;
        auto visit = [&](int b, uint32_t sv, int& j) {
            if (j == 0 && b >= min_size && n - b >= min_size) {
                int64_t d = (int64_t)n * (int64_t)run - (int64_t)tot * (int64_t)b;
                double sc = score_f64(d, (uint64_t)b * (uint64_t)(n - b));
                if (sc >= best) { second = best; best = sc; best_b = b; }
                else if (sc > second) second = sc;
            }
            run += (uint64_t)sv;
            if (++j == jump) j = 0;
        };
        int j = 0;
        if (in_regs) {
            TPS_UNROLL
            for (int i = 0; i < CHUNK_REGS; ++i)
                if (lo + i < hi) visit(lo + i, (uint32_t)S[lo + i], j);
        } else {
            for (int b = lo; b < hi; ++b) visit(b, (uint32_t)S[b], j);
        }
        uint64_t bits = 0;
        if (best >= 0.0) __builtin_memcpy(&bits, &best, 8);
        wg_max_bits(bits, (uint64_t*)&misc[M_MAXSC]);
    }
    TPS_SYNC();
    TPS_PHASE {
        const double best = TPS_AT(best_), second = TPS_AT(second_);
        const int best_b = TPS_AT(best_b_);
        double m;
        __builtin_memcpy(&m, &misc[M_MAXSC], 8);
        const double thr = m * (1.0 - 1e-14);
        uint32_t near = (best >= thr && best >= 0.0 ? 1u : 0u) + (second >= thr && second >= 0.0 ? 1u : 0u);
        if (near) lds_add(&misc[M_NTIE], near);
        if (best == m && best_b >= 0) lds_max_i32((int32_t*)&misc[M_BESTB], best_b);
    }
    TPS_SYNC();
    tie = misc[M_NTIE] > 1u;
    if (tie) {
        Cand ex = binseg_exact_wg(S, n, jump, min_size, xs);
        bkp = ex.b;
        gain = ex.b < 0 ? 0.0 : gain_from((int64_t)ex.d, ex.den, n, n_patterns);
    } else {
        bkp = (int32_t)misc[M_BESTB];
        double m;
        __builtin_memcpy(&m, &misc[M_MAXSC], 8);
        gain = bkp < 0 ? 0.0 : m / (double)n / ((double)n_patterns * (double)n_patterns);
        TPS_SYNC();
    }
}

template <typename ST>
TPS_DEV void binseg_from_lc(const ScanArgs& a, const Lds& l, uint64_t lc_g, const ST* S_global, int n, uint64_t tot, int jump,
                            int min_size, int n_patterns, uint32_t* misc, uint32_t* xs, int& bkp, double& gain, bool& tie) {
    const int ncand = (n - 1) / jump;
    Lane<double> best_(-1.0);
    Lane<int> best_b_(-1);
    Lane<bool> amb_(false);
    Lane<uint64_t> bits_(0);
    const int c_min = (min_size + jump - 1) / jump > 1 ? (min_size + jump - 1) / jump : 1;
    const int c_max = (n - min_size) / jump < ncand ? (n - min_size) / jump : ncand;
    const bool exact53 = (double)n * 4294967296.0 < 9007199254740992.0 && (double)tot * (double)n < 9007199254740992.0;
    const double nf = (double)n, totf = (double)tot;
    const bool int_d = (double)tot * (double)n < 2147483648.0 && tot < (1ull << 24);
    constexpr int LCV = 16;
    const bool prefilter = exact53 && c_max - c_min < LCV * NT;
    int nslot = c_max >= c_min ? (c_max - c_min + NT) / NT : 0;
    TPS_PIN_S(nslot);
    Lane<float> p_s1_(-1.0f), p_s2_(-1.0f);
    Lane<uint32_t> p_lc_(0);
    Lane<int> p_c_(-1);
    float thr32 = -1.0f;
    bool crowded = false;
    TPS_ISA_REGION(5);
    if (prefilter) {
        auto prefilter_phase = [&](auto intd_) {
        TPS_PHASE {
            constexpr bool INTD = decltype(intd_)::value != 0;
            float &p_s1 = TPS_AT(p_s1_), &p_s2 = TPS_AT(p_s2_);
            uint32_t& p_lc = TPS_AT(p_lc_);
            p_s1 = -1.0f; p_s2 = -1.0f; p_lc = 0;
            int p_j = -1;
            const int c0 = c_min + tid;
            const uint32_t off0 = 4u * (uint32_t)c0;
            const float nf32 = (float)n, bstep = (float)(NT * jump);
            float bf = (float)(c0 * jump);
            const uint32_t ntb_step = 0u - (uint32_t)tot * (uint32_t)(NT * jump);
            uint32_t ntb = 0u - (uint32_t)tot * (uint32_t)(c0 * jump);
            auto slot = [&](int j, uint32_t lc, auto last_) {
                float d32;
                if constexpr (INTD) {
                    d32 = (float)(int32_t)(mul24((uint32_t)n, lc) + ntb);
                    ntb += ntb_step;
                } else {
                    d32 = (float)__builtin_fma(-totf, (double)bf, nf * (double)lc);
                }
                const float den32 = bf * (nf32 - bf);
                bf += bstep;
                float s_ = d32 * d32 * rcp_f32(den32);
                if constexpr (decltype(last_)::value != 0) s_ = tid <= c_max - c_min - j * NT ? s_ : -1.0f;
                const bool gt = s_ > p_s1;
                p_s2 = med3_f32(p_s1, p_s2, s_);
                p_lc = gt ? lc : p_lc;
                p_j = gt ? j : p_j;
                p_s1 = gt ? s_ : p_s1;
            };
            auto group = [&](int g, auto checked_) {
                constexpr bool CHECKED = decltype(checked_)::value != 0;
                uint32_t lcv[4];
                TPS_UNROLL
                for (int i = 0; i < 4; ++i) {
                    const uint32_t joff = 4u * NT * (uint32_t)(4 * g + i);
                    if constexpr (CHECKED) lcv[i] = g32_load_at(lc_g, off0 + joff < 4u * (uint32_t)c_max ? off0 + joff : 4u * (uint32_t)c_max);
                    else lcv[i] = g32_load_at(lc_g + joff, off0);
                }
                TPS_UNROLL
                for (int i = 0; i < 4; ++i) slot(4 * g + i, lcv[i], checked_);
            };
            if constexpr (INTD) {
                if (nslot > 4) group(0, IntC<0>()); else if (nslot > 0) group(0, IntC<1>());
                if (nslot > 8) group(1, IntC<0>()); else if (nslot > 4) group(1, IntC<1>());
                if (nslot > 12) group(2, IntC<0>()); else if (nslot > 8) group(2, IntC<1>());
                if (nslot > 12) group(3, IntC<1>());
            } else {
                if (nslot > 0) group(0, IntC<1>());
                if (nslot > 4) group(1, IntC<1>());
                if (nslot > 8) group(2, IntC<1>());
                if (nslot > 12) group(3, IntC<1>());
            }
            TPS_AT(p_c_) = p_j >= 0 ? c0 + p_j * NT : -1;
        }
        };
        if (int_d) {
            prefilter_phase(IntC<1>());
        } else {
            TPS_EMU_COUNT(11);
// ... 207 lines not shown
                TPS_SYNC();
            }
            TPS_STAMP(3);
            TPS_PHASE { trc_sum_packed(a, l, st_s, st_e, r, tid); }
        } else {
            TPS_EMU_COUNT(14);
            TPS_PHASE { for (int i = tid; i < HIST_DW; i += NT) l.blk[i] = 0; }
            TPS_SYNC();
            if (plain) {
                TPS_PHASE { trc_count_thread<true>(a, l, st_s, st_e, tid); }
            } else {
                TPS_PHASE { trc_count_thread<false>(a, l, st_s, st_e, tid); }
            }
            TPS_SYNC();
            TPS_STAMP(3);
            TPS_PHASE { trc_sum_thread(a, l, st_s, st_e, r, tid); }
        }
        if (!decided) {
            TPS_SYNC();
            ks = uniform(l.misc[M_BEST]);
            ke = uniform(l.misc[M_BEST + 1]);
        }
        res.best_start = (int32_t)(ks >> 5); res.best_start_idx = 31 - (int32_t)(ks & 31u);
        res.best_end = (int32_t)(ke >> 5); res.best_end_idx = 31 - (int32_t)(ke & 31u);
        tail = res.best_start > res.best_end ? 0 : 1;
        int best = tail ? res.best_end : res.best_start;
        pass = (L > prm.min_len && best > prm.min_count) ? 1 : 0;
    } else if (a.tails_in) {
        uint8_t tv = a.tails_in[r];
        tail = tv & 1;
        pass = (tv & 2) ? 0 : 1;
    }
    res.tail = tail;
    res.pass = pass;
    TPS_STAMP(4);

    int n_win = 0;
    uint64_t s_total = 0;
    if (pass && (prm.flags & TPS_F_WINDOWS)) {
        const int64_t m = L < prm.maxlen ? L : prm.maxlen;
        const int64_t n_s = m - prm.trimfirst;
        if (n_s >= prm.window) n_win = (int)((n_s - prm.window) / prm.slide) + 1;
        if (n_win / prm.jump + 1 > a.lc_cap) n_win = 0;
        const int64_t out_base = a.win_off ? a.win_off[r] : 0;
        if constexpr (SV == 0) {
            const uint64_t lc_gen = a.lc_global ? (uint64_t)(uintptr_t)(a.lc_scratch + r * (int64_t)a.lc_stride) : 0ull;
            const int blk_per_tile = a.spans_per_tile << a.blk_log2;
            const int tw = blk_per_tile - a.q - 1;
            for (int w0 = 0; w0 < n_win; w0 += tw) {
                const int nw_tile = (n_win - w0) < tw ? (n_win - w0) : tw;
                const int64_t i0 = (int64_t)w0 * prm.slide;
                int64_t n_stage = n_s - i0;
                const int64_t cap = (int64_t)blk_per_tile * prm.slide + 32;
                if (n_stage > cap) n_stage = cap;
                const Stage st = stage_plan(a.seq2, a.inv, woff, L, tail == 1, prm.trimfirst, i0, (int)n_stage);
                const int blk_need = nw_tile + a.q + 1;
                const int spans = (blk_need + (1 << a.blk_log2) - 1) >> a.blk_log2;
                const int ndw = spans * a.span_dw + 8 < a.seq_dw ? spans * a.span_dw + 8 : a.seq_dw;
                TPS_PHASE { if (tid == 0) l.misc[M_INVALID] = 0; }
                TPS_SYNC();
                TPS_PHASE { stage_thread(st, has_inv, l.seq2, l.val, (ndw + 3) >> 2, &l.misc[M_INVALID], tid); }
                TPS_SYNC();
                if (w0 == 0) TPS_STAMP(5);
                TPS_PHASE {
                    for (int sp = tid; sp < spans; sp += NT) blocks_span(a, l, st.delta, sp);
                }
                TPS_SYNC();
                if (w0 == 0) TPS_STAMP(6);
                wg_exclusive_scan(l.Tot, spans, &l.misc[M_SCAN]);
                if (w0 == 0) TPS_STAMP(7);
                for (int base = 0; base < nw_tile; base += WIN_U * NT) {
                    TPS_PHASE { windows_group(a, l, st.delta, w0, nw_tile, out_base, base, tid); }
                    TPS_SYNC();
                    const uint32_t gsum = wg_exclusive_scan(l.row, WIN_U * NT, &l.misc[M_SCAN]);
                    TPS_PHASE { candidates_group(a, l, lc_gen, w0, nw_tile, base, (uint32_t)s_total, tid); }
                    s_total += gsum;
                    TPS_SYNC();
                }
                if (w0 == 0) TPS_STAMP(8);
            }
        } else {
            typedef TileGeo<SV ? SV : 1, FULL> t_;
            constexpr int PF = t_::PF;
            const TileConst tc = tile_const(a, r);
            int tw = (int)uniform((uint32_t)a.tw);
            TPS_PIN_S(tw);
            bool pp = false;
            if constexpr (RAW) pp = a.pp_d >= 0 && (SO ? a.pp_d > 0 : (a.pp_d == 0 && a.raw != nullptr));
            bool pp_expect = a.so_fast != 2;
            auto tile_stage = [&](int w0_) {
                const int64_t i0 = (int64_t)w0_ * prm.slide;
                int64_t n_stage = n_s - i0;
                int64_t cap = (int64_t)t_::BASES;
                const int64_t need = (int64_t)(tw - 1 + tc.q) * prm.slide + tc.r + 13;
                if (cap > need) cap = need;
                const int ns32 = (int)n_stage, cap32 = (int)cap;
                const int n_st = ns32 > cap32 ? cap32 : ns32;
                return stage_plan(a.seq2, a.inv, woff, L, tail == 1, prm.trimfirst, i0, n_st);
            };
            LaneArr<u32x4, PF> pf_;
            LaneArr<u32x2, PF> pv_;
            TPS_LANES { for (int u = 0; u < PF; ++u) TPS_AT(pv_)[u].x = TPS_AT(pv_)[u].y = 0; }
            const bool rv = tail == 1;
            constexpr bool ORIENT = !RAW && !SO && PF == 1;
            Lane<uint32_t> pf_off(0);
            if constexpr (ORIENT) {
                TPS_LANES {
                    TPS_AT(pf_off) = stage_lane_off(rv, tid);
                    TPS_PIN_V(TPS_AT(pf_off));
                }
            }
            auto pf_load = [&](const Stage& stn, int tid) {
                u32x4* const pf = TPS_AT(pf_);
                u32x2* const pv = TPS_AT(pv_);
                TPS_UNROLL
                for (int u = 0; u < PF; ++u) {
                    const int c = tid + u * NT;
                    pf[u].x = pf[u].y = pf[u].z = pf[u].w = 0;
                    if constexpr (!ORIENT) pv[u].x = pv[u].y = 0;
                    if (c < stn.nq) {
                        const uint32_t off = ORIENT ? TPS_AT(pf_off) : stage_lane_off(rv, tid);
                        pf[u] = load16(stage_base(stn, u * NT) + off);
                        if (has_inv) pv[u] = load8(stage_inv_base(stn, u * NT) + (off >> 1));
                    }
                }
            };
            TPS_ISA_REGION(1);
            if (n_win > 0) {
                const Stage st0 = tile_stage(0);
                TPS_PHASE {
                    if (tid == 0) { l.misc[M_INVALID] = 0; l.misc[M_NTIE] = 0; }
                    pf_load(st0, tid);
                }
            }
            for (int w0 = 0, tile = 0; w0 < n_win; w0 += tw, ++tile) {
                const int nw_tile = (n_win - w0) < tw ? (n_win - w0) : tw;
                TPS_ISA_REGION(2);
                const Stage st = tile_stage(w0);
                TPS_PHASE {
                    const u32x4* const pf = TPS_AT(pf_);
                    const u32x2* const pv = TPS_AT(pv_);
                    TPS_UNROLL
                    for (int u = 0; u < PF; ++u) {
                        const int c = tid + u * NT;
                        if (c < t_::NQ) {
                            if constexpr (!ORIENT) lds_store16(l.seq2 + SEQ_LEAD + 4 * c, stage_orient(st, pf[u]));
                            else if (rv) lds_store16(l.seq2 + SEQ_LEAD + 4 * c, stage_reversed(pf[u]));
                            else lds_store16(l.seq2 + SEQ_LEAD + 4 * c, pf[u]);
                            if (has_inv) {
                                u32x2 o;
                                o.x = o.y = 0;
                                if (!ORIENT || c < st.nq) o = stage_orient_inv(st, pv[u]);
                                if (o.x | o.y) l.misc[M_INVALID] = 1u;
                                lds_store8((uint32_t*)l.val + (SEQ_LEAD >> 1) + 2 * c, o);
                            }
                        }
                    }
                    if (tid == NT - 1) {
                        u32x4 z;
                        z.x = z.y = z.z = z.w = 0;
                        lds_store16(l.seq2, z);
                        if (has_inv) { u32x2 z2; z2.x = z2.y = 0; lds_store8((uint32_t*)l.val, z2); }
                    }
                }
                TPS_SYNC();
                TPS_ISA_REGION(3);
                if (w0 + tw < n_win) {
// ... 13 lines not shown
                            if (a.so_fast && !pp_expect) {
                                if (home) chained = tile_pp_s<SP, 0, HD, F16K, HR>(a, tc, l, fdelta, w0, tile, nw_tile, out_base, s_total);
                                else switch (a.pp_d) {
                                    case 2: chained = tile_pp_s<SP, 0, 2, F16K>(a, tc, l, fdelta, w0, tile, nw_tile, out_base, s_total); break;
                                    case 3: chained = tile_pp_s<SP, 0, 3, F16K>(a, tc, l, fdelta, w0, tile, nw_tile, out_base, s_total); break;
                                    case 4: chained = tile_pp_s<SP, 0, 4, F16K>(a, tc, l, fdelta, w0, tile, nw_tile, out_base, s_total); break;
                                    case 5: chained = tile_pp_s<SP, 0, 5, F16K>(a, tc, l, fdelta, w0, tile, nw_tile, out_base, s_total); break;
                                    default: chained = tile_pp_s<SP, 0, (SP < 6 ? SP : 6), F16K>(a, tc, l, fdelta, w0, tile, nw_tile, out_base, s_total); break;
                                }
                            }
                            if (!chained) { pp_expect = false; continue; }
                            const uint64_t s_before = s_total;
                            if (home) tile_pp_s<SP, HD, 0, F16K, HR>(a, tc, l, fdelta, w0, tile, nw_tile, out_base, s_total);
                            else switch (a.pp_d) {
                                case 2: tile_pp_s<SP, 2, 0, F16K>(a, tc, l, fdelta, w0, tile, nw_tile, out_base, s_total); break;
                                case 3: tile_pp_s<SP, 3, 0, F16K>(a, tc, l, fdelta, w0, tile, nw_tile, out_base, s_total); break;
                                case 4: tile_pp_s<SP, 4, 0, F16K>(a, tc, l, fdelta, w0, tile, nw_tile, out_base, s_total); break;
                                case 5: tile_pp_s<SP, 5, 0, F16K>(a, tc, l, fdelta, w0, tile, nw_tile, out_base, s_total); break;
                                default: tile_pp_s<SP, (SP < 6 ? SP : 6), 0, F16K>(a, tc, l, fdelta, w0, tile, nw_tile, out_base, s_total); break;
                            }
                            pp_expect = a.so_fast != 2 && (s_total - s_before) > (uint64_t)nw_tile * (uint64_t)(pat.P + 4);
                        } else {
                            constexpr int HR4 = 96 % SP;
                            if constexpr (PAIR && (HR4 & 1) == 0) {
                                if (tc.r == HR4 && a.pair_n != 0) { tile_pp_s<SP, 0, 0, false, HR4, true>(a, tc, l, fdelta, w0, tile, nw_tile, out_base, s_total); continue; }
                            }
                            if (tc.r == HR4) tile_pp_s<SP, 0, 0, false, HR4>(a, tc, l, fdelta, w0, tile, nw_tile, out_base, s_total);
                            else tile_pp_s<SP, 0>(a, tc, l, fdelta, w0, tile, nw_tile, out_base, s_total);
                        }
                        continue;
                    }
                    if (pp && SO) {
                        TPS_PHASE { if (tid == 0) l.misc[M_SCAN + 6] = 1u; }
                        TPS_SYNC();
                    }
                }
                if constexpr (SO && !RAW) {
                    constexpr int SP = SV ? SV : 5;
                    if (a.pp_d > 0 && uniform(l.misc[M_INVALID]) == 0) {
                        bool done = false;
#define TPS_LC_CD_RP(D_, N) case N: if constexpr (N < SP && D_ <= SP) { tile_lc_s<SP, false, (N < SP ? N : 0), false, false, (D_ <= SP ? D_ : 0)>(a, tc, l, fdelta, w0, tile, nw_tile, out_base, s_total, r); done = true; } break;
#define TPS_LC_CD(D_) case D_: switch (tc.r) { TPS_LC_CD_RP(D_, 0) TPS_LC_CD_RP(D_, 1) TPS_LC_CD_RP(D_, 2) TPS_LC_CD_RP(D_, 3) TPS_LC_CD_RP(D_, 4) TPS_LC_CD_RP(D_, 5) TPS_LC_CD_RP(D_, 6) TPS_LC_CD_RP(D_, 7) default: break; } break;
                        if (a.so_fast) {
                            if constexpr (DCLASS == 1) { switch (a.pp_d) { TPS_LC_CD(2) TPS_LC_CD(3) TPS_LC_CD(4) default: break; } }
                            else if constexpr (DCLASS == 2) { switch (a.pp_d) { TPS_LC_CD(5) TPS_LC_CD(6) default: break; } }
                            else { switch (a.pp_d) { TPS_LC_CD(2) TPS_LC_CD(3) TPS_LC_CD(4) TPS_LC_CD(5) TPS_LC_CD(6) default: break; } }
                        }
#undef TPS_LC_CD
#undef TPS_LC_CD_RP
                        if (done) continue;
                    }
                }
                constexpr int SF = SV ? SV : 1;
                constexpr bool LC = !SO && !RAW;
                if (uniform(l.misc[M_INVALID]) != 0) {
                    if constexpr (LC) tile_lc_s<SF, true, -1, false, false, 0, P16K>(a, tc, l, fdelta, w0, tile, nw_tile, out_base, s_total, r);
                    else tile_fused_s<SF, SO, true, -1, RAW>(a, tc, l, fdelta, w0, tile, nw_tile, out_base, s_total, r);
                } else if constexpr (SO || RAW) {
                    if (tc.r == 0) tile_fused_s<SF, SO, false, 0, RAW>(a, tc, l, fdelta, w0, tile, nw_tile, out_base, s_total, r);
                    else tile_fused_s<SF, SO, false, -1, RAW>(a, tc, l, fdelta, w0, tile, nw_tile, out_base, s_total, r);
                } else {
#define TPS_TILE_RP(N) case N: if constexpr (N < SF) { if ((tc.q & 7) == 0) tile_lc_s<SF, false, (N < SF ? N : 0), PAIR, true, 0, P16K>(a, tc, l, fdelta, w0, tile, nw_tile, out_base, s_total, r); \
                                                       else tile_lc_s<SF, false, (N < SF ? N : 0), PAIR, false, 0, P16K>(a, tc, l, fdelta, w0, tile, nw_tile, out_base, s_total, r); } break;
                    switch (tc.r) {
                        TPS_TILE_RP(0) TPS_TILE_RP(1) TPS_TILE_RP(2) TPS_TILE_RP(3) TPS_TILE_RP(4) TPS_TILE_RP(5) TPS_TILE_RP(6) TPS_TILE_RP(7)
                        TPS_TILE_RP(8) TPS_TILE_RP(9) TPS_TILE_RP(10) TPS_TILE_RP(11)
                        default: break;
                    }
#undef TPS_TILE_RP
                }
                if (w0 == 0) TPS_STAMP(8);
            }
        }
    }
    res.n_win = n_win;
    TPS_STAMP(9);

    if (n_win > 0 && (prm.flags & TPS_F_BINSEG) && binseg_admissible(n_win, prm.jump, prm.min_size)) {
        int bkp;
        double gain;
        bool tie = false;
        TPS_FENCE_WG();
        const uint64_t lc_g = a.lc_global ? (uint64_t)(uintptr_t)(a.lc_scratch + r * (int64_t)a.lc_stride) : 0ull;
        if constexpr (SV != 0)
            binseg_from_lc(a, l, lc_g, (const uint16_t*)(a.sums16 + (a.win_off16 ? a.win_off16[r] : 0)), n_win, s_total, prm.jump, prm.min_size, pat.P,
                           l.misc, l.blk, bkp, gain, tie);
        else
            binseg_from_lc(a, l, lc_g, (const int32_t*)(a.sums + (a.win_off ? a.win_off[r] : 0)), n_win, s_total, prm.jump, prm.min_size, pat.P,
                           l.misc, l.blk, bkp, gain, tie);
        res.bkp = bkp;
        res.gain = gain;
        res.flags = tie ? TPS_RES_TIE : 0u;
    }
    TPS_PHASE { if (tid == 0) a.results[r] = res; }
    TPS_STAMP(10);
}

constexpr int BINSEG_SMEM_DW = ((XS_DW + 2 + MISC_DW + NT + 3) / 4) * 4;
TPS_DEV void binseg_read(const BinsegArgs& a, int64_t r, uint32_t* smem) {
    const int64_t lo = a.win_off[r];
    const int n = (int)(a.win_off[r + 1] - lo);
    const int32_t* S = a.sums + lo;
    uint32_t* xs = smem;
    uint32_t* misc = smem + ((XS_DW + 1) / 2) * 2;
    uint32_t* bs = misc + MISC_DW;
    int bkp = -1;
    double gain = 0.0;
    bool tie = false;
    if (binseg_admissible(n, a.jump, a.min_size)) {
        binseg_wg(S, n, a.jump, a.min_size, a.n_patterns, bs, misc, xs, bkp, gain, tie);
    }
    TPS_PHASE {
        if (tid == 0) {
            a.bkp[r] = bkp;
            if (a.gain) a.gain[r] = gain;
            if (a.tie) a.tie[r] = tie ? 1 : 0;
        }
    }
}

struct StrideArgs {
    const tps_read_result* base_results;
    const uint16_t* base_sums16;
    const int64_t* base_win_off16;
    const uint8_t* base_raw;
    const int64_t* base_win_off;
    const int64_t* win_off;
    int32_t* sums;
    uint8_t* raw;
    tps_read_result* results;
    int64_t n_reads;
    int32_t m, P, n_patterns, jump, min_size, binseg;
    int32_t s16_dw;
};
TPS_DEV void stride_read(const StrideArgs& a, int64_t r, uint32_t* smem, uint16_t* s16) {
    tps_read_result res = a.base_results[r];
    const int64_t lo = a.win_off[r];
    const int n = res.n_win > 0 ? (int)(a.win_off[r + 1] - lo) : 0;
    const int64_t lo16 = a.base_win_off16[r], lob = a.base_win_off[r];
    const int m = a.m, P = a.P;
    TPS_PHASE {
        for (int w = tid; w < n; w += NT) {
            const uint32_t v = a.base_sums16[lo16 + (int64_t)w * m];
            a.sums[lo + w] = (int32_t)v;
            if (s16) s16[w] = (uint16_t)v;
        }
        if (a.raw) {
            if ((P & 3) == 0) {
                const int pd = P >> 2;
                const uint32_t* src = (const uint32_t*)a.base_raw + lob * pd;
                uint32_t* dst = (uint32_t*)a.raw + lo * pd;
                for (int w = tid; w < n; w += NT) {
                    const uint32_t* sr = src + (int64_t)w * m * pd;
                    uint32_t* dr = dst + (int64_t)w * pd;
                    TPS_NOVEC
                    for (int d = 0; d < pd; ++d) dr[d] = sr[d];
                }
            } else {
                const uint8_t* src = a.base_raw + lob * P;
                uint8_t* dst = a.raw + lo * P;
                for (int w = tid; w < n; w += NT) {
                    const uint8_t* sr = src + (int64_t)w * m * P;
                    uint8_t* dr = dst + (int64_t)w * P;
                    TPS_NOVEC
                    for (int d = 0; d < P; ++d) dr[d] = sr[d];
                }
            }
// ... 134 lines not shown
```

### topsicle_amd/csrc/tps_plan.h

```cpp
#pragma once
#include <cstdlib>
#include <algorithm>
#include <cstdint>
#include <cstring>
#include <string>
#include <vector>

#include "tps_device.h"

namespace tps {

inline int64_t window_count(int64_t L, int W, int s, int t, int M) {
    int64_t m = std::min<int64_t>(L, M);
    int64_t ns = m - t;
    if (W < 1 || s < 1 || ns < W) return 0;
    return (ns - W) / s + 1;
}

inline void plan_dispatch_order(const int64_t* n_win, const uint8_t* passes, int64_t n, std::vector<int32_t>& order) {
    order.clear();
    if (n < 2 || n > 0x7FFFFFFFll) return;
    constexpr int NCLS = 64;
    int64_t mx = 0;
    for (int64_t i = 0; i < n; ++i) if (passes[i] && n_win[i] > mx) mx = n_win[i];
    if (mx == 0) return;
    auto cls = [&](int64_t i) -> int { return passes[i] ? (int)(1 + (n_win[i] * (NCLS - 2) + mx - 1) / mx) : 0; };
    int64_t cnt[NCLS + 1] = {0};
    for (int64_t i = 0; i < n; ++i) ++cnt[cls(i)];
    int used = 0;
    for (int c = 0; c < NCLS; ++c) used += cnt[c] != 0;
    if (used < 2) return;
    int64_t start[NCLS];
    int64_t acc = 0;
    for (int c = NCLS - 1; c >= 0; --c) { start[c] = acc; acc += cnt[c]; }
    order.resize((size_t)n);
    for (int64_t i = 0; i < n; ++i) order[(size_t)start[cls(i)]++] = (int32_t)i;
}

inline int64_t sums16_slots(int64_t nw) { return (nw + 7) & ~7ll; }

struct BatchLayout {
    std::vector<int64_t> win_off;
    std::vector<int64_t> win_off16;
    std::vector<int32_t> order;
    int64_t max_nwin = 0;
    int64_t max_len = 0;
};
inline void plan_batch_layout(const int64_t* offsets, int64_t n, const tps_params& prm, BatchLayout& lay) {
    lay.win_off.resize((size_t)n + 1);
    lay.win_off16.resize((size_t)n + 1);
    lay.max_nwin = lay.max_len = 0;
    std::vector<int64_t> nwv((size_t)n);
    std::vector<uint8_t> longer((size_t)n);
    int64_t acc = 0, acc16 = 0;
    for (int64_t i = 0; i < n; ++i) {
        lay.win_off[(size_t)i] = acc;
        lay.win_off16[(size_t)i] = acc16;
        const int64_t len = offsets[i + 1] - offsets[i];
        const int64_t nw = window_count(len, prm.window, prm.slide, prm.trimfirst, prm.maxlen);
        lay.max_len = std::max(lay.max_len, len);
        lay.max_nwin = std::max(lay.max_nwin, nw);
        acc += nw;
        acc16 += sums16_slots(nw);
        nwv[(size_t)i] = (prm.flags & TPS_F_WINDOWS) ? nw : 0;
        longer[(size_t)i] = !(prm.flags & TPS_F_STEP1) || len > prm.min_len;
    }
    lay.win_off[(size_t)n] = acc;
    lay.win_off16[(size_t)n] = acc16;
    plan_dispatch_order(nwv.data(), longer.data(), n, lay.order);
}

inline void widen_sums16(const uint16_t* src16, const int64_t* win_off16, const int64_t* win_off, int64_t r0, int64_t r1, int32_t* dst) {
    for (int64_t i = r0; i < r1; ++i) {
        const uint16_t* s = src16 + (win_off16[i] - win_off16[r0]);
        int32_t* d = dst + (win_off[i] - win_off[r0]);
        const int64_t cnt = win_off[i + 1] - win_off[i];
        for (int64_t w = 0; w < cnt; ++w) d[w] = (int32_t)s[w];
    }
}

inline int64_t clear_skipped_windows(const tps_read_result* results, const int64_t* win_off, int64_t n, int64_t scale, size_t unit,
                                     int64_t lo, int64_t hi, void* buf) {
    if (hi <= lo || n <= 0) return 0;
    int64_t a = 0, b = n;
    while (a < b) {
        const int64_t mid = a + (b - a) / 2;
        if (win_off[mid + 1] * scale <= lo) a = mid + 1; else b = mid;
    }
    int64_t cleared = 0;
    for (int64_t i = a; i < n && win_off[i] * scale < hi; ++i) {
        if (results[i].pass) continue;
        const int64_t x = std::max(win_off[i] * scale, lo), y = std::min(win_off[i + 1] * scale, hi);
        if (y > x) {
            memset((char*)buf + (size_t)(x - lo) * unit, 0, (size_t)(y - x) * unit);
            cleared += y - x;
        }
    }
    return cleared;
}

inline int gcd_i(int a, int b) { while (b) { int t = a % b; a = b; b = t; } return a; }

inline std::string build_patterns(const char* pats, int P, int k, std::vector<uint32_t>& lut, PatInfo& pi) {
    if (k < 1 || k > TPS_MAX_K) return "k=" + std::to_string(k) + " not supported (1.." + std::to_string(TPS_MAX_K) + ")";
    if (P < 1 || P > TPS_MAX_PATTERNS) return std::to_string(P) + " patterns not supported (1.." + std::to_string(TPS_MAX_PATTERNS) + ")";
    const bool hashed = k > TPS_DIRECT_K;
    if (!hashed) lut.assign((size_t)1 << (2 * k), 0u);
    pi = PatInfo{};
    pi.P = P;
    pi.k = k;
    pi.kmask = (1u << (2 * k)) - 1u;
    pi.all_mask = (1u << P) - 1u;
    uint32_t per_pat[16] = {0, 0, 0, 0, 0, 0, 0, 0, 0, 0, 0, 0, 0, 0, 0, 0};
    std::vector<uint32_t> code_mask((size_t)P, 0u);
    std::vector<uint32_t> codes((size_t)P);
    for (int p = 0; p < P; ++p) {
        uint32_t code = 0;
        char up[16];
        for (int i = 0; i < k; ++i) {
            char ch = pats[p * k + i];
            if (ch >= 'a' && ch <= 'z') ch = (char)(ch - 32);
            up[i] = ch;
            uint32_t v;
            switch (ch) {
                case 'A': v = 0; break;
                case 'C': v = 1; break;
                case 'T': v = 2; break;
                case 'G': v = 3; break;
                default: return "pattern " + std::to_string(p) + " has a non-ACGT letter";
            }
            code |= v << (2 * i);
        }
        if (!hashed) lut[code] |= 1u << p;
        codes[(size_t)p] = code;
        for (int d = 1; d < k; ++d) {
            bool periodic = true;
            for (int i = 0; i + d < k; ++i) periodic = periodic && (up[i] == up[i + d]);
            if (periodic) { per_pat[d] |= 1u << p; pi.so_mask |= 1u << p; }
        }
    }
    for (int p = 0; p < P; ++p)
        for (int o = 0; o < P; ++o)
            if (codes[(size_t)o] == codes[(size_t)p]) code_mask[(size_t)p] |= 1u << o;
    for (int p = 0; p < P; ++p)
        if (code_mask[(size_t)p] & (code_mask[(size_t)p] - 1)) pi.dup_mask |= 1u << p;
    if (hashed) {
        const int log2h = 8;
        const uint32_t H = 1u << log2h;
        uint32_t mul = 0;
        for (uint32_t cand = 0x9E3779B1u, tries = 0; tries < 200000 && !mul; ++tries, cand += 0xC657CB56u) {
            const uint32_t m = cand | 1u;
            std::vector<int> owner(H, -1);
// ... 37 lines not shown
    auto waves_per_cu = [&](int w) {
        a.wpg = w;
        const int64_t dw = wg_lds_dwords(a);
        if (dw > budget_dw) return 0;
        const int64_t gran = std::max<int64_t>(1, (dw * 4 + 1279) / 1280);
        const int64_t wgs = std::min<int64_t>(std::min<int64_t>(8, 128 / gran), (4 * max_waves_simd) / w);
        return (int)std::min<int64_t>(32, wgs * w);
    };
    int best = WPG, best_w = waves_per_cu(WPG);
    if (lut_dw(a) * 4 >= 8192 || (a.pair16 && (a.pair_n + lut_dw(a)) * 4 >= 8192)) {
        const int v = waves_per_cu(WPG_MAX);
        if (v > best_w) { best = WPG_MAX; best_w = v; }
    }
    a.wpg = best;
}


inline bool has_specialised_slide(int s) { return s == 5 || s == 6 || s == 7 || s == 8; }
inline bool has_default_only_slide(int s) { return s == 3 || s == 4 || (s >= 9 && s <= 12); }

struct PlanKnobs {
    int spans_per_tile = 0;
    int force_generic = 0;
    int force_pair = 0;
    int so_order = 0;
    int wpg = 0;
};

inline std::string plan_geometry_core(ScanArgs& a, const tps_params& prm, int k, int P, int64_t max_nwin, int64_t budget_dw, const PlanKnobs& kn);
inline std::string plan_geometry(ScanArgs& a, const tps_params& prm, int k, int P, int64_t max_nwin, int64_t budget_dw,
                                 const PlanKnobs& kn = PlanKnobs()) {
    a.wpg = WPG;
    std::string err = plan_geometry_core(a, prm, k, P, max_nwin, budget_dw, kn);
    if (err.empty() && a.variant && !a.pat.hash_shift) {
        const int64_t single_bytes = (int64_t)a.lut_n * (a.lut16 ? 2 : 4);
        if ((single_bytes & (single_bytes - 1)) != 0 || ((int64_t)a.pair_n * 4) % single_bytes != 0)
            err = "LDS plan: the single table (" + std::to_string(single_bytes) + " B) would not be aligned behind a pair table of " + std::to_string((int64_t)a.pair_n * 4) + " B";
    }
    if (err.empty()) {
        const bool raw = (prm.flags & TPS_F_STORE_RAW) != 0;
        plan_wpg(a, budget_dw, !a.variant ? 8 : raw ? 5 : a.pat.so_mask != 0 ? 6 : 8);
        if ((kn.wpg == WPG || kn.wpg == WPG_MAX) && a.variant) {
            const int32_t keep = a.wpg;
            a.wpg = kn.wpg;
            if (wg_lds_dwords(a) > budget_dw) a.wpg = keep;
        }
    }
    return err;
}
inline std::string plan_geometry_core(ScanArgs& a, const tps_params& prm, int k, int P, int64_t max_nwin, int64_t budget_dw, const PlanKnobs& kn) {
    const int spans_pref = kn.spans_per_tile, force_generic = kn.force_generic;
    a.lut_n = a.pat.hash_shift ? 2 * 256 : 1 << (2 * k);
    a.lw = std::max(0, prm.window - k);
    a.q = a.lw / prm.slide;
    a.r = a.lw % prm.slide;
    if (max_nwin > 500000) return "too many windows per read (" + std::to_string(max_nwin) + ")";
    {
        int min_per = k;
        for (int i = 0; i < a.pat.n_periods; ++i) min_per = std::min(min_per, std::max(1, (int)a.pat.period[i]));
        const int64_t occ_max = a.lw > 0 ? (a.lw - 1) / min_per + 1 : 0;
        if ((prm.flags & TPS_F_STORE_RAW) && occ_max > 255)
            return "raw counts are bytes: a pattern can occur " + std::to_string(occ_max) + " times in a window of " +
                   std::to_string(prm.window) + " (max 255); use a smaller --windowSize with --rawcountpattern";
        const int64_t sw_max = (int64_t)P * ((a.lw + k - 1) / k + 1);
        if (max_nwin * sw_max >= (1ll << 32)) return "window sums of one read exceed 32 bits (windows per read x window size too large)";
        if ((double)max_nwin * (double)max_nwin * (double)max_nwin * (double)sw_max >= 147573952589676412928.0 )
            return "change-point arithmetic would exceed 128 bits (windows per read x window size too large)";
    }
    const int jump = std::max(prm.jump, 1);
    a.lc_cap = (int)(max_nwin / jump + 2);
    a.jump_magic = jump == 1 ? 0u : (uint32_t)(((1ull << 32) + (uint64_t)jump - 1) / (uint64_t)jump);
    a.head_dw = 4 * ((prm.no_bp + 63 + 63) / 64) + 4;
    int max_period = 0;
    for (int i = 0; i < a.pat.n_periods; ++i) max_period = std::max(max_period, a.pat.period[i]);
    const bool sw16_ok = (int64_t)P * ((a.lw + k - 1) / k + 1) < 65536;
    const int one_period = (a.pat.dup_mask == 0 && k >= 4 && a.pat.n_periods == 1 && a.pat.period[0] >= 2 && 2 * a.pat.period[0] >= k) ? a.pat.period[0] : 0;
    const bool p16_ok = P == 16 && a.pat.dup_mask == 0 && !(prm.flags & TPS_F_STORE_RAW) &&
                        (a.pat.so_mask == 0 || (!a.val_on && one_period > 0 && one_period <= prm.slide && a.lw <= 255));
    const bool fused = !force_generic && spans_pref <= 0 && k <= TPS_DIRECT_K && (has_specialised_slide(prm.slide) || (has_default_only_slide(prm.slide) && a.pat.so_mask == 0 && !(prm.flags & TPS_F_STORE_RAW))) &&
                       (P <= 15 || p16_ok) && a.q >= 8 && sw16_ok &&
                       a.q / 8 + 2 < (XLANES - NT) && max_period <= std::min(prm.slide, 6) &&
                       2 * a.head_dw <= fused_seq_dw(prm.slide);
    a.tw = 0; a.pair_n = 0; a.lc_global = 0; a.lc_stride = 0; a.pp_d = -1; a.so_fast = 0; a.seq_alias = 0; a.lut_fields = 0; a.tile_full = 0;
    a.lut16 = 0; a.xt_alias = 0; a.xt_own = 0; a.pair16 = 0;
    if (fused) {
        const bool pp_counts = a.pat.dup_mask == 0 && k >= 4 && P <= 14 && (8 * prm.slide + k - 1) / k <= 14 && (prm.slide + k - 1) / k <= 2 &&
                               a.lw / k + 2 <= 127;
        if (pp_counts && a.pat.n_periods == 0) a.pp_d = 0;
        if (pp_counts && a.pat.n_periods == 1 && a.pat.period[0] >= 2 && 2 * a.pat.period[0] >= k) a.pp_d = a.pat.period[0];
        if (!(prm.flags & TPS_F_STORE_RAW) && P > 14 && one_period > 0) a.pp_d = one_period;
        a.lut_fields = (a.pp_d >= 0 && (prm.flags & TPS_F_STORE_RAW)) ? 1 : 0;
        a.so_fast = kn.so_order == 2 ? 2 : 1;
        if (!(prm.flags & TPS_F_STORE_RAW) && a.pp_d > 0 && a.lw > 255) a.so_fast = 0;
        if (a.pat.so_mask != 0 && !(prm.flags & TPS_F_STORE_RAW)) {
            a.lut16 = 1;
            a.xt_alias = 2;
            a.xt_own = (a.val_on || !a.so_fast || a.pp_d <= 0) ? 1 : 0;
        }
        if (prm.flags & TPS_F_STORE_RAW) {
            if (a.lut_fields && a.pat.so_mask != 0 && a.pp_d > 0 && a.lut_n >= 4096) a.lut16 = 1;
            a.xt_alias = 2;
            a.xt_own = (a.val_on || (a.pat.so_mask != 0 ? a.pp_d <= 0 : a.pp_d != 0)) ? 1 : 0;
        }
        if (a.pat.so_mask == 0 && !(prm.flags & TPS_F_STORE_RAW)) { a.xt_alias = 2; a.xt_own = 0; }
        a.variant = prm.slide;
        a.blk_log2 = 3;
        a.span_dw = 0;
        a.spans_per_tile = NT;
        a.nblk_cap = NT * 8;
        a.rec_rs = 0;
        a.tot_dw = 4;
        a.tile_full = 1;
        a.seq_dw = fused_seq_dw(prm.slide);
        a.seq_alias = 0;
#ifndef TPS_EMU
        if (a.pat.so_mask == 0 && !(prm.flags & TPS_F_STORE_RAW)) a.seq_alias = 1;
#endif
        a.tw = ((int)NT * 8 - a.q - 1) & ~1;
        a.lc_global = 1;
        a.lc_stride = 2 * ((a.lc_cap + 1) & ~1);
        a.pair_n = (a.pat.so_mask == 0 && k <= 4 && !(prm.flags & TPS_F_STORE_RAW)) ? (1 << (2 * (k + 1))) : 0;
        if (a.pat.so_mask == 0 && k <= 4 && (prm.flags & TPS_F_STORE_RAW) && a.lut_fields && a.pp_d == 0 && prm.slide == 6 && a.r == 0) a.pair_n = 1 << (2 * (k + 1));
        a.pair16 = 0;
        if (a.pat.so_mask == 0 && a.pat.dup_mask == 0 && k == 5 && P <= 15 && has_specialised_slide(prm.slide) && !(prm.flags & TPS_F_STORE_RAW)) {
            a.pair16 = 1;
            a.lut16 = 1;
            a.pair_n = (1 << (2 * (k + 1))) / 2;
        }
        a.blk_dw = (int32_t)blk_region_dw(a);
        if (a.pair_n && !kn.force_pair) {
            auto waves_per_cu = [&](int w) {
                const int32_t w0 = a.wpg;
                a.wpg = w;
                const int64_t dw = wg_lds_dwords(a);
                a.wpg = w0;
                if (dw > budget_dw) return 0;
                return (int)(std::min<int64_t>(8, 128 / std::max<int64_t>(1, (dw * 4 + 1279) / 1280)) * w);
            };
            const int with_pair = a.pair16 ? std::max(waves_per_cu(WPG), waves_per_cu(WPG_MAX)) : waves_per_cu(WPG);
            const int32_t keep = a.pair_n;
            const int32_t keep16 = a.pair16;
            a.pair_n = 0;
            if (keep16) { a.lut16 = 0; a.pair16 = 0; }
            if (with_pair >= 5 * WPG || waves_per_cu(WPG) <= with_pair) { a.pair_n = keep; if (keep16) { a.pair16 = 1; a.lut16 = 1; } }
        }
        if (wg_lds_dwords(a) <= budget_dw) return "";
        a.tw = 0; a.pair_n = 0; a.lc_global = 0; a.lc_stride = 0; a.pp_d = -1; a.so_fast = 0; a.seq_alias = 0; a.lut_fields = 0;
        a.lut16 = 0; a.xt_alias = 0; a.xt_own = 0; a.pair16 = 0;
    }
    a.variant = 0;
    a.lc_global = 1;
    a.lc_stride = 2 * ((a.lc_cap + 1) & ~1);
    const int g = gcd_i(prm.slide, 16);
    a.span_dw = prm.slide / g;
    const int bps = 16 / g;
    a.blk_log2 = 0;
    while ((1 << a.blk_log2) < bps) ++a.blk_log2;
    const int max_spans = 2 * NT;
    const int min_spans = (a.q + 2 + bps - 1) / bps;
    const int64_t need_blk = max_nwin + a.q + 1;
    const int need_spans = (int)std::min<int64_t>((need_blk + bps - 1) / bps, max_spans);
    int spans = spans_pref > 0 ? std::min(spans_pref, max_spans) : std::min(std::max(need_spans, 1), (int)NT);
    spans = std::max(min_spans, std::min(spans, std::max(need_spans, 1)));
    if (spans > max_spans) return "window/slide combination needs " + std::to_string(spans) + " spans per tile (max " + std::to_string(max_spans) + ")";
    auto fill = [&](int sp) {
        a.spans_per_tile = sp;
        a.nblk_cap = sp * bps;
        a.rec_rs = 0;
        a.tot_dw = std::max(((sp + 2) / 2) * 2, (int)NT);
        a.seq_dw = (std::max(sp * a.span_dw + 8, 2 * a.head_dw) + 3) & ~3;
        a.blk_dw = (int32_t)blk_region_dw(a);
        return wg_lds_dwords(a);
    };
    if (spans_pref > 0) {
        if (fill(spans) > budget_dw)
            return "LDS plan does not fit with " + std::to_string(spans) + " spans per tile";
        return "";
    }
    while (fill(spans) > budget_dw) {
        if (spans <= min_spans)
            return "LDS plan does not fit: window=" + std::to_string(prm.window) + " slide=" + std::to_string(prm.slide) +
                   " k=" + std::to_string(k) + " windows/read=" + std::to_string(max_nwin);
        spans = std::max(min_spans, spans / 2);
    }
    return "";
}

template <typename F>
inline int stride_base(const ScanArgs& planned, const tps_params& prm, int k, int P, F max_nwin_of, int64_t budget_dw, const PlanKnobs& kn) {
    if (planned.variant != 0 || kn.force_generic || kn.spans_per_tile > 0 || !(prm.flags & TPS_F_WINDOWS)) return 0;
    for (int s0 = 12; s0 >= 3; --s0) {
        if (prm.slide <= s0 || prm.slide % s0 != 0 || prm.slide / s0 > 6) continue;
        if (!has_specialised_slide(s0) && !has_default_only_slide(s0)) continue;
        ScanArgs t{};
        t.val_on = planned.val_on;
        t.pat = planned.pat;
        tps_params pb = prm;
        pb.slide = s0;
        pb.flags = (prm.flags | TPS_F_STORE_SUMS) & ~(uint32_t)TPS_F_BINSEG;
        if (plan_geometry(t, pb, k, P, max_nwin_of(s0), budget_dw, kn).empty() && t.variant != 0) return s0;
    }
    return 0;
}

}
```

### topsicle_amd/csrc/tps_wave.h

```cpp
#pragma once
#include <stdint.h>

#ifdef TPS_EMU
#define TPS_DEV static inline
#define TPS_HD static inline
#define TPS_AT(x) ((x).v[tid])
#define TPS_PHASE for (int tid = 0; tid < tps::NT; ++tid)
#define TPS_LANES for (int tid = 0; tid < tps::NT; ++tid)
#define TPS_PHASE_WITH(ln) for (int tid = (ln) * 0; tid < tps::NT; ++tid)
#define TPS_SYNC() ((void)0)
#define TPS_FENCE_WG() ((void)0)
#define TPS_UNROLL
#define TPS_NOVEC
#define TPS_PIN_S(x) ((void)0)
#define TPS_PIN_V(x) ((void)0)
#else
#define TPS_DEV __device__ __forceinline__
#define TPS_HD __host__ __device__ inline
#define TPS_AT(x) (x)
__device__ __forceinline__ int tps_fresh_lane() {
    int t = (int)(threadIdx.x & 63u);
    asm volatile("" : "+v"(t));
    return t;
}
#define TPS_PHASE for (int tid = tps_fresh_lane(), once_ = 1; once_; once_ = 0)
#define TPS_LANES for (int tid = (int)(threadIdx.x & 63u), once_ = 1; once_; once_ = 0)
#define TPS_PHASE_WITH(ln) if (const int tid = (ln); true)
#define TPS_SYNC() do { __builtin_amdgcn_fence(__ATOMIC_SEQ_CST, "wavefront"); __builtin_amdgcn_wave_barrier(); } while (0)
#define TPS_FENCE_WG() __builtin_amdgcn_fence(__ATOMIC_SEQ_CST, "workgroup")
#define TPS_UNROLL _Pragma("unroll")
#define TPS_NOVEC _Pragma("clang loop vectorize(disable) interleave(disable) unroll(disable)")
#define TPS_PIN_S(x) asm volatile("" : "+s"(x))
#define TPS_PIN_V(x) asm volatile("" : "+v"(x))
#endif

#if defined(TPS_ISA_MARKS) && !defined(TPS_EMU)
#define TPS_STAMP(i) asm volatile(";tps_stamp %0" ::"i"(i))
#define TPS_ISA_MARK(id) asm volatile(";tps_mark %0" ::"i"(id))
#define TPS_ISA_REGION(id) asm volatile(";tps_region %0" ::"i"(id))
#elif defined(TPS_EMU) || !defined(TPS_STAMPS)
#define TPS_STAMP(i) ((void)0)
#define TPS_ISA_MARK(id) ((void)(id))
#define TPS_ISA_REGION(id) ((void)(id))
#else
#define TPS_STAMP(i) do { if (a.stamps && (threadIdx.x & 63u) == 0) a.stamps[r * 16 + (i)] = __builtin_readcyclecounter(); } while (0)
#define TPS_ISA_MARK(id) ((void)(id))
#define TPS_ISA_REGION(id) ((void)(id))
#endif
#if defined(TPS_EMU) || !defined(TPS_STAMPS)
#define TPS_PP_STAMP(i) ((void)0)
#else
#define TPS_PP_STAMP(i) do { if (w0 == 0 && a.stamps && (threadIdx.x & 63u) == 0) a.stamps[tc.rd * 16 + (i)] = __builtin_readcyclecounter(); } while (0)
#endif

namespace tps {

constexpr int NT = 64;

#ifdef TPS_EMU
constexpr int EMU_COUNTERS = 16;
inline int& emu_counter(int i) { static int c[EMU_COUNTERS] = {0}; return c[i]; }
#define TPS_EMU_COUNT(i) ((void)++tps::emu_counter(i))
#define TPS_EMU_COUNT_N(i, n) ((void)(tps::emu_counter(i) += (int)(n)))
TPS_DEV int tps_fresh_lane() { return 0; }
#else
#define TPS_EMU_COUNT(i) ((void)0)
#define TPS_EMU_COUNT_N(i, n) ((void)0)
#endif

#ifdef TPS_EMU
template <typename T>
struct Lane {
    T v[NT];
    Lane() {}
    Lane(T x) { for (int t = 0; t < NT; ++t) v[t] = x; }
};
template <typename T, int N>
struct LaneArr {
    T v[NT][N];
};
#else
template <typename T> using Lane = T;
template <typename T, int N> using LaneArr = T[N];
#endif

#ifdef TPS_EMU
TPS_DEV uint64_t wave_ballot(const Lane<bool>& p) {
    uint64_t m = 0;
    for (int t = 0; t < NT; ++t) m |= (uint64_t)(p.v[t] ? 1 : 0) << t;
    return m;
}
#else
TPS_DEV uint64_t wave_ballot(const Lane<bool>& p) { return __builtin_amdgcn_ballot_w64(p); }
#endif
#ifdef TPS_EMU
TPS_DEV Lane<uint32_t> wave_incl_sum(const Lane<uint32_t>& x) {
    Lane<uint32_t> r;
    uint32_t acc = 0;
    for (int t = 0; t < NT; ++t) { acc += x.v[t]; r.v[t] = acc; }
    return r;
// ... 207 lines not shown
TPS_DEV uint32_t g16_load(uint64_t base, uint32_t i) {
    typedef const __attribute__((address_space(1))) uint16_t* gp_t;
    return ((gp_t)(uintptr_t)base)[i];
}
TPS_DEV uint32_t g32_load_at(uint64_t base, uint32_t byte_off) {
    typedef const __attribute__((address_space(1))) uint8_t* gb_t;
    typedef const __attribute__((address_space(1))) uint32_t* gp_t;
    return *(gp_t)((gb_t)(uintptr_t)base + byte_off);
}
TPS_DEV void g32_store(uint64_t base, uint32_t i, uint32_t v) {
    typedef __attribute__((address_space(1))) uint32_t* gp_t;
    ((gp_t)(uintptr_t)base)[i] = v;
}
TPS_DEV uint32_t g32_load(uint64_t base, uint32_t i) {
    typedef const __attribute__((address_space(1))) uint32_t* gp_t;
    return ((gp_t)(uintptr_t)base)[i];
}
#endif

TPS_DEV uint32_t mulhi32(uint32_t x, uint32_t y) { return (uint32_t)(((uint64_t)x * (uint64_t)y) >> 32); }
TPS_DEV uint32_t mul24(uint32_t x, uint32_t y) { return (x & 0xFFFFFFu) * (y & 0xFFFFFFu); }
#ifdef TPS_EMU
TPS_DEV uint32_t add_bytes(uint32_t v, uint32_t acc) { return acc + (v & 255u) + ((v >> 8) & 255u) + ((v >> 16) & 255u) + (v >> 24); }
#else
TPS_DEV uint32_t add_bytes(uint32_t v, uint32_t acc) { return __builtin_amdgcn_sad_u8(v, 0u, acc); }
#endif

#ifdef TPS_EMU
TPS_DEV uint32_t xor3(uint32_t a, uint32_t b, uint32_t c) { return a ^ b ^ c; }
TPS_DEV uint32_t maj3(uint32_t a, uint32_t b, uint32_t c) { return (a & b) | (c & (a | b)); }
TPS_DEV uint32_t or_and(uint32_t a, uint32_t b, uint32_t c) { return (a | b) & c; }
#else
TPS_DEV uint32_t xor3(uint32_t a, uint32_t b, uint32_t c) { return __builtin_amdgcn_bitop3_b32(a, b, c, 0x96); }
TPS_DEV uint32_t maj3(uint32_t a, uint32_t b, uint32_t c) { return __builtin_amdgcn_bitop3_b32(a, b, c, 0xE8); }
TPS_DEV uint32_t or_and(uint32_t a, uint32_t b, uint32_t c) { return __builtin_amdgcn_bitop3_b32(a, b, c, 0xA8); }
#endif

#ifdef TPS_EMU
TPS_DEV uint32_t pk_u16_sub(uint32_t a, uint32_t b) { return ((a - b) & 0xFFFFu) | (((a >> 16) - (b >> 16)) << 16); }
TPS_DEV uint32_t pk_u16_add(uint32_t a, uint32_t b) { return ((a + b) & 0xFFFFu) | (((a >> 16) + b) << 16); }
#else
typedef unsigned short tps_u16x2 __attribute__((ext_vector_type(2)));
TPS_DEV tps_u16x2 as_u16x2(uint32_t v) { return __builtin_bit_cast(tps_u16x2, v); }
TPS_DEV uint32_t pk_u16_sub(uint32_t a, uint32_t b) { return __builtin_bit_cast(uint32_t, as_u16x2(a) - as_u16x2(b)); }
TPS_DEV uint32_t pk_u16_add(uint32_t a, uint32_t b) { return __builtin_bit_cast(uint32_t, as_u16x2(a) + (tps_u16x2)((unsigned short)b)); }
#endif

#ifdef TPS_EMU
TPS_DEV u32x4 lds_load16(const uint32_t* p) { u32x4 v; v.x = p[0]; v.y = p[1]; v.z = p[2]; v.w = p[3]; return v; }
TPS_DEV void lds_store16(uint32_t* p, const u32x4& v) { p[0] = v.x; p[1] = v.y; p[2] = v.z; p[3] = v.w; }
TPS_DEV void lds_store8(uint32_t* p, const u32x2& v) { p[0] = v.x; p[1] = v.y; }
#else
TPS_DEV u32x4 lds_load16(const uint32_t* p) { return *(const u32x4*)p; }
TPS_DEV void lds_store16(uint32_t* p, const u32x4& v) { *(u32x4*)p = v; }
TPS_DEV void lds_store8(uint32_t* p, const u32x2& v) { *(u32x2*)p = v; }
#endif

constexpr int STORE_AUX = 2;
#ifdef TPS_EMU
TPS_DEV void g_store_sw8(uint16_t* tile_out, int lane, int nw_tile, const uint32_t* v) {
    for (int i = 0; i < 8; ++i)
        if (8 * lane + i < nw_tile) tile_out[8 * lane + i] = (uint16_t)v[i];
}
TPS_DEV void g_store_sw8p(uint16_t* tile_out, int lane, int nw_tile, const uint32_t* p) {
    for (int i = 0; i < 8; ++i)
        if (8 * lane + i < nw_tile) tile_out[8 * lane + i] = (uint16_t)(p[i >> 1] >> (16 * (i & 1)));
}
#else
TPS_DEV void g_store_sw8(uint16_t* tile_out, int lane, int nw_tile, const uint32_t* v) {
    typedef unsigned int v4u __attribute__((ext_vector_type(4)));
    const __amdgpu_buffer_rsrc_t rs = __builtin_amdgcn_make_buffer_rsrc((void*)tile_out, 0, ((nw_tile + 1) & ~1) * 2, 0x00020000);
    v4u t;
    t.x = v[0] | (v[1] << 16); t.y = v[2] | (v[3] << 16); t.z = v[4] | (v[5] << 16); t.w = v[6] | (v[7] << 16);
    __builtin_amdgcn_raw_buffer_store_b128(t, rs, lane * 16, 0, STORE_AUX);
}
TPS_DEV void g_store_sw8p(uint16_t* tile_out, int lane, int nw_tile, const uint32_t* p) {
    typedef unsigned int v4u __attribute__((ext_vector_type(4)));
    const __amdgpu_buffer_rsrc_t rs = __builtin_amdgcn_make_buffer_rsrc((void*)tile_out, 0, ((nw_tile + 1) & ~1) * 2, 0x00020000);
    v4u t;
    t.x = p[0]; t.y = p[1]; t.z = p[2]; t.w = p[3];
    __builtin_amdgcn_raw_buffer_store_b128(t, rs, lane * 16, 0, STORE_AUX);
}
#endif
#ifdef TPS_EMU
TPS_DEV void g_store16_clamped(uint32_t* base, int n_dw, int cdw, const u32x4& t) {
    const uint32_t v[4] = {t.x, t.y, t.z, t.w};
    for (int i = 0; i < 4; ++i)
        if (cdw + i < n_dw) base[cdw + i] = v[i];
}
#else
TPS_DEV void g_store16_clamped(uint32_t* base, int n_dw, int cdw, const u32x4& t) {
    typedef unsigned int v4u __attribute__((ext_vector_type(4)));
    const __amdgpu_buffer_rsrc_t rs = __builtin_amdgcn_make_buffer_rsrc((void*)base, 0, n_dw * 4, 0x00020000);
    v4u x;
    x.x = t.x; x.y = t.y; x.z = t.z; x.w = t.w;
    __builtin_amdgcn_raw_buffer_store_b128(x, rs, cdw * 4, 0, STORE_AUX);
}
#endif
#ifdef TPS_EMU
TPS_DEV void g32_store_clamped(uint64_t base, uint32_t n, uint32_t i, uint32_t v) {
    if (i < n) ((uint32_t*)(uintptr_t)base)[i] = v;
}
#else
TPS_DEV void g32_store_clamped(uint64_t base, uint32_t n, uint32_t i, uint32_t v) {
    const __amdgpu_buffer_rsrc_t rs = __builtin_amdgcn_make_buffer_rsrc((void*)(uintptr_t)base, 0, (int)(n * 4u), 0x00020000);
    __builtin_amdgcn_raw_buffer_store_b32(v, rs, (int)(i * 4u), 0, 0);
}
#endif

}
```

### topsicle_amd/hiplib.py

```python
from __future__ import annotations

import ctypes as C
import os

import numpy as np

LIB_NAME = "libtopsicle_hip.so"
LIB_PATH = os.path.join(os.path.dirname(os.path.abspath(__file__)), LIB_NAME)

F_STEP1, F_WINDOWS, F_BINSEG, F_STORE_SUMS, F_STORE_RAW, F_TAILS_IN = 1, 2, 4, 8, 16, 32
MAX_K, MAX_PATTERNS, MAX_SLOTS = 15, 31, 16
WIDE_MAX_K, WIDE_MAX_PATTERNS = 32, 64
FOLLOW_MAX_FWD, FOLLOW_WIDE_MAX_FWD, FOLLOW_HIST_MAX = 15, 32, 8

EXPORTS = [
    "tps_abi_version", "tps_device_count", "tps_ctx_create", "tps_ctx_destroy", "tps_last_error",
    "tps_set_patterns", "tps_set_patterns_wide", "tps_batch_upload", "tps_batch_upload_packed", "tps_batch_upload_nib4", "tps_batch_share", "tps_host_alloc", "tps_host_free",
    "tps_batch_download_packed", "tps_batch_kmer_followers", "tps_batch_kmer_followers_wide", "tps_batch_motif_census", "tps_batch_variant_census", "tps_batch_tract_map", "tps_batch_end_sketch", "tps_sketch_links", "tps_batch_end_window", "tps_window_offsets", "tps_window_place", "tps_batch_adapter_find", "tps_batch_set_tails", "tps_batch_scan", "tps_sync",
    "tps_batch_results", "tps_batch_window_offsets", "tps_batch_window_sums", "tps_batch_window_raw",
    "tps_batch_raw_to_fd", "tps_batch_trc_counts", "tps_trc_counts", "tps_window_counts", "tps_binseg_l2", "tps_binseg_l2_ties", "tps_batch_read_sums", "tps_window_count",
    "tps_kernel_time_ms", "tps_kernel_time_reset", "tps_device_info", "tps_batch_kernel_info", "tps_ctx_debug_option", "tps_debug_stamps_get",
]


class TopsicleHipError(RuntimeError):
    pass


class Params(C.Structure):
    _fields_ = [("no_bp", C.c_int32), ("min_len", C.c_int32), ("min_count", C.c_int32),
                ("window", C.c_int32), ("slide", C.c_int32), ("trimfirst", C.c_int32),
                ("maxlen", C.c_int32), ("jump", C.c_int32), ("min_size", C.c_int32),
                ("flags", C.c_uint32)]


DESC_DTYPE = np.dtype([("word_off", "<i8"), ("len", "<i4"), ("flags", "<u4")], align=True)
assert DESC_DTYPE.itemsize == 16
RD_HAS_INVALID = 1

NIB_SRC_DTYPE = np.dtype([("off", "<i8"), ("flags", "<u4"), ("reserved", "<u4")], align=True)
assert NIB_SRC_DTYPE.itemsize == 16
NIB_REVERSE = 1

RESULT_DTYPE = np.dtype([("best_start", "<i4"), ("best_start_idx", "<i4"), ("best_end", "<i4"),
                         ("best_end_idx", "<i4"), ("tail", "<i4"), ("pass", "<i4"), ("n_win", "<i4"),
                         ("bkp", "<i4"), ("gain", "<f8"), ("flags", "<u4"), ("reserved", "<u4")], align=True)
assert RESULT_DTYPE.itemsize == 48
MOTIF_HIT_DTYPE = np.dtype([("unit", "<u8"), ("period", "<i4"), ("support", "<i4"), ("run_start", "<i4"), ("run_len", "<i4"),
                            ("n_bases", "<i4"), ("reserved", "<i4")], align=True)
assert MOTIF_HIT_DTYPE.itemsize == 32
MOTIF_MAX_PERIOD, MOTIF_MAX_SPAN = 32, 4096
VARIANT_MAX_UNIT, VARIANT_BIN_RANGE, VARIANT_MAX_BINS = 32, (64, 4064), 64
TRACT_DTYPE = np.dtype([("begin", "<i4"), ("end", "<i4"), ("hits", "<i4"), ("blocks", "<i4")])
assert TRACT_DTYPE.itemsize == 16
TRACT_UNIT_RANGE, TRACT_BLOCK_RANGE, TRACT_GAP_RANGE, TRACT_MIN_BLOCKS_RANGE, TRACT_MAX_TRACTS_RANGE = (4, 32), (64, 1024), (0, 64), (1, 64), (1, 16)
ENDS_K_RANGE, ENDS_BUCKETS, ENDS_MAX_WINDOW, LINKS_MAX_N, LINKS_MAX_LINKS = (8, 16), (64, 128, 256, 512), 16384, 262144, 256
ENDS_EMPTY = 0xFFFFFFFF
ANCHOR_MAX_SPAN, ANCHOR_MAX_ROWS = 4096, 262144
PLACE_MAX_REFS, PLACE_MAX_OCC = 1024, 64
ADAPTER_LEN_RANGE, ADAPTER_MAX_PATTERNS, ADAPTER_MAX_REGION = (12, 64), 64, 1024
RES_TIE = 1


def make_params(no_bp=1000, min_len=0, min_count=-1, window=100, slide=6, trimfirst=100, maxlen=20000,
                jump=5, min_size=2, flags=F_STEP1 | F_WINDOWS | F_BINSEG) -> Params:
    return Params(no_bp, min_len, min_count, window, slide, trimfirst, maxlen, jump, min_size, flags)


_lib = None


def load_library(path: str | None = None) -> C.CDLL:
    global _lib
    if _lib is not None and path is None:
        return _lib
    p = path or os.environ.get("TOPSICLE_HIP_LIB") or LIB_PATH
    if not os.path.exists(p):
        raise TopsicleHipError(f"{p} not found: build the HIP library first (python -c 'import __graft_entry__ as g; g.build()'). "
                               "topsicle_amd has no CPU fallback.")
    try:
        lib = C.CDLL(p)
    except OSError as e:
        raise TopsicleHipError(f"cannot load {p}: {e}") from e
    vp, i32, i64 = C.c_void_p, C.c_int32, C.c_int64
    proto = {
        "tps_abi_version": (C.c_int, []),
        "tps_device_count": (C.c_int, [C.POINTER(C.c_int)]),
        "tps_ctx_create": (C.c_int, [C.c_int, C.POINTER(vp)]),
        "tps_ctx_destroy": (C.c_int, [vp]),
        "tps_last_error": (C.c_char_p, []),
        "tps_set_patterns": (C.c_int, [vp, C.c_char_p, i32, i32]),
        "tps_set_patterns_wide": (C.c_int, [vp, C.c_char_p, i32, i32]),
        "tps_batch_upload": (C.c_int, [vp, i32, vp, vp, i64]),
        "tps_batch_upload_packed": (C.c_int, [vp, i32, vp, vp, vp, i64, i64]),
        "tps_batch_upload_nib4": (C.c_int, [vp, i32, vp, i64, vp, vp, i64, i64]),
        "tps_batch_share": (C.c_int, [vp, i32, vp, i32]),
        "tps_host_alloc": (C.c_int, [vp, i64, C.POINTER(vp)]),
        "tps_host_free": (C.c_int, [vp, vp]),
        "tps_batch_download_packed": (C.c_int, [vp, i32, vp, vp, vp, i64, i64, C.POINTER(i64)]),
        "tps_batch_kmer_followers": (C.c_int, [vp, i32, i32, i32, i32, i32, i32, vp, i64, vp, i64]),
        "tps_batch_kmer_followers_wide": (C.c_int, [vp, i32, i32, i32, i32, i32, i32, vp, i64, vp, i64]),
        "tps_batch_motif_census": (C.c_int, [vp, i32, i32, i32, i32, i32, i32, vp, i64, vp, i64]),
        "tps_batch_variant_census": (C.c_int, [vp, i32, C.c_uint64, i32, vp, vp, vp, i64, i32, i32, vp, i64, vp, i64]),
        "tps_batch_tract_map": (C.c_int, [vp, i32, C.c_uint64, i32, i32, i32, i32, i32, i32, vp, i64, vp, i64, vp, i64]),
        "tps_batch_end_sketch": (C.c_int, [vp, i32, C.c_uint64, i32, i32, i32, vp, vp, vp, i64, vp, i64, vp, i64]),
        "tps_sketch_links": (C.c_int, [vp, vp, i64, i32, i64, i32, i32, vp, i64, vp, i64, vp, i64]),
        "tps_batch_end_window": (C.c_int, [vp, i32, C.c_uint64, i32, i32, vp, vp, vp, i64, i32, vp, i64, vp, i64]),
        "tps_window_offsets": (C.c_int, [vp, vp, vp, vp, vp, i64, i32, i32, vp, vp, vp, i64]),
        "tps_window_place": (C.c_int, [vp, vp, i64, vp, i64, vp, i64, vp, i64, vp, i64, vp, i32, i32, i32, i32, vp, vp, vp, vp, vp, vp, vp, i64]),
        "tps_batch_adapter_find": (C.c_int, [vp, i32, vp, vp, i32, vp, vp, vp, i64, vp, i64]),
        "tps_batch_set_tails": (C.c_int, [vp, i32, vp]),
        "tps_batch_scan": (C.c_int, [vp, i32, C.POINTER(Params)]),
        "tps_sync": (C.c_int, [vp]),
        "tps_batch_results": (C.c_int, [vp, i32, vp, i64]),
        "tps_batch_window_offsets": (C.c_int, [vp, i32, vp, i64]),
        "tps_batch_window_sums": (C.c_int, [vp, i32, vp, i64]),
        "tps_batch_window_raw": (C.c_int, [vp, i32, vp, i64]),
        "tps_batch_raw_to_fd": (C.c_int, [vp, i32, vp, i64, C.c_int, i64, vp, C.POINTER(C.c_uint32), C.POINTER(i64)]),
        "tps_batch_trc_counts": (C.c_int, [vp, i32, vp, vp, i64]),
        "tps_trc_counts": (C.c_int, [vp, vp, vp, i64, i32, vp, vp]),
        "tps_window_counts": (C.c_int, [vp, vp, vp, vp, i64, i32, i32, i32, i32, vp, vp, vp]),
        "tps_binseg_l2": (C.c_int, [vp, vp, vp, i64, i32, i32, i32, vp, vp]),
        "tps_binseg_l2_ties": (C.c_int, [vp, vp, vp, i64, i32, i32, i32, vp, vp, vp]),
        "tps_batch_read_sums": (C.c_int, [vp, i32, i64, vp, i64]),
        "tps_window_count": (i64, [i64, i32, i32, i32, i32]),
        "tps_kernel_time_ms": (C.c_int, [vp, C.POINTER(i32), C.POINTER(C.c_double), C.POINTER(C.c_double)]),
        "tps_kernel_time_reset": (C.c_int, [vp]),
        "tps_device_info": (C.c_int, [vp, C.c_char_p, i32]),
        "tps_batch_kernel_info": (C.c_int, [vp, i32, C.c_char_p, i32]),
        "tps_ctx_debug_option": (C.c_int, [vp, C.c_char_p, i64]),
        "tps_debug_stamps_get": (C.c_int, [vp, i32, vp, i64]),
    }
    for name, (res, args) in proto.items():
        try:
            fn = getattr(lib, name)
        except AttributeError as e:
            raise TopsicleHipError(f"{p} does not export {name}") from e
        fn.restype, fn.argtypes = res, args
    if path is None:
        _lib = lib
    return lib


def _ptr(a):
    return None if a is None else a.ctypes.data_as(C.c_void_p)


def needs_wide(patterns) -> bool:
    return bool(patterns) and (len(patterns[0]) > MAX_K or len(patterns) > MAX_PATTERNS)


def set_table(engine, patterns):
    if needs_wide(patterns):
        engine.set_patterns_wide(patterns)
    else:
        engine.set_patterns(patterns)


def debug_options_from_env() -> dict:
    out = {}
    for item in os.environ.get("TOPSICLE_HIP_DEBUG", "").split(","):
        item = item.strip()
        if item:
            key, _, val = item.partition("=")
            out[key.strip()] = int(val) if val.strip() else 1
    return out


_crc_cb = None


def _crc32_callback():
    global _crc_cb
    if _crc_cb is None:
        from . import seqio
        lib = seqio._load_io()
        if lib is None:
            raise TopsicleHipError("libtopsicle_io.so is not built (its tps_crc32 checksums the raw-count archive)")
        _crc_cb = C.cast(lib.tps_crc32, C.c_void_p)
    return _crc_cb


def pack_reads(seqs) -> tuple[np.ndarray, np.ndarray]:
    bs = [s.encode("ascii", "replace") if isinstance(s, str) else bytes(s) for s in seqs]
    offsets = np.zeros(len(bs) + 1, dtype=np.int64)
    if bs:
        np.cumsum([len(b) for b in bs], out=offsets[1:])
    bases = np.frombuffer(b"".join(bs), dtype=np.uint8) if bs else np.zeros(0, np.uint8)
    return np.ascontiguousarray(bases), offsets


def window_count(read_len: int, window: int, slide: int, trimfirst: int, maxlen: int) -> int:
    ns = min(read_len, maxlen) - trimfirst
    if window < 1 or slide < 1 or ns < window:
        return 0
    return (ns - window) // slide + 1


def binseg_l2_float64(y, jump: int = 5, min_size: int = 2):
    sig = np.asarray(y, dtype=np.float64).reshape(-1, 1)
    n = sig.shape[0]
    if (n // jump) < 1 or (-(-min_size // jump)) * jump + min_size > n:
        return -1

    def cost(a, b):
        return sig[a:b].var(axis=0).sum() * (b - a)

    whole = cost(0, n)
    best = None
    for b in range(0, n, jump):
        if b >= min_size and n - b >= min_size:
            cand = (whole - cost(0, b) - cost(b, n), b)
            if best is None or cand > best:
                best = cand
    return -1 if best is None else int(best[1])


def resolve_ties(engine, slot: int, res: np.ndarray, n_patterns: int, jump: int = 5, min_size: int = 2) -> int:
    if "flags" not in res.dtype.names:
        return 0
    idx = np.nonzero((res["flags"] & RES_TIE) != 0)[0]
    for i in idx:
        s_w = engine.read_sums(slot, int(i), int(res["n_win"][i]))
        res["bkp"][i] = binseg_l2_float64(np.asarray(s_w, dtype=np.float64) / n_patterns, jump, min_size)
    return len(idx)


def _region(tails, begin, end, call):
    tails = np.ascontiguousarray(tails, dtype=np.uint8)
    begin = np.ascontiguousarray(begin, dtype=np.int32)
    end = np.ascontiguousarray(end, dtype=np.int32)
    if not (len(tails) == len(begin) == len(end)):
        raise TopsicleHipError(f"{call}: tails, begin and end must have one entry per read")
    return tails, begin, end


class HipScanner:

    def __init__(self, device: int = 0, lib_path: str | None = None):
        self.lib = load_library(lib_path)
        n = C.c_int(0)
        rc = self.lib.tps_device_count(C.byref(n))
        if rc != 0 or n.value <= 0:
            raise TopsicleHipError("no MI355X / HIP device visible: " + self._err() + " (topsicle_amd has no CPU fallback)")
        h = C.c_void_p()
        self._check(self.lib.tps_ctx_create(int(device), C.byref(h)))
        self._h = h
        self.device = int(device)
        self.patterns: list[str] = []
        self._n = {}
        self._lib_path = lib_path
        self._helpers: list["HipScanner"] = []
        for key, value in debug_options_from_env().items():
            self.debug_option(key, value)

    def debug_option(self, key: str, value: int = 1):
        self._check(self.lib.tps_ctx_debug_option(self._h, key.encode(), int(value)))
        self._debug = getattr(self, "_debug", {})
        self._debug[key] = int(value)
        for h in self._helpers:
            h.debug_option(key, value)

    def stamps(self, slot: int) -> np.ndarray:
        n = self._n[slot]
        out = np.zeros((n, 16), dtype=np.uint64)
        self._check(self.lib.tps_debug_stamps_get(self._h, slot, _ptr(out), n))
        return out

    def helper(self, j: int) -> "HipScanner":
        while len(self._helpers) <= j:
            h = HipScanner(self.device, self._lib_path)
            for key, value in getattr(self, "_debug", {}).items():
                h.debug_option(key, value)
            self._helpers.append(h)
        return self._helpers[j]

    def _err(self) -> str:
        m = self.lib.tps_last_error()
        return m.decode("utf-8", "replace") if m else ""

    def _check(self, rc: int):
        if rc != 0:
            raise TopsicleHipError(f"libtopsicle_hip error {rc}: {self._err()}")

    def close(self):
        for h in getattr(self, "_helpers", []):
            h.close()
        self._helpers = []
        if getattr(self, "_h", None):
            self.lib.tps_ctx_destroy(self._h)
            self._h = None

    def __del__(self):
        try:
            self.close()
        except Exception:
            pass

    def __enter__(self):
        return self

    def __exit__(self, *exc):
        self.close()

    def device_info(self) -> str:
        buf = C.create_string_buffer(256)
        self._check(self.lib.tps_device_info(self._h, buf, 256))
        return buf.value.decode()

    def kernel_info(self, slot: int) -> str:
        buf = C.create_string_buffer(256)
        self._check(self.lib.tps_batch_kernel_info(self._h, slot, buf, 256))
        return buf.value.decode()

    def set_patterns(self, patterns: list[str]):
        if not patterns:
            raise TopsicleHipError("empty pattern list")
        k = len(patterns[0])
        if any(len(p) != k for p in patterns):
            raise TopsicleHipError("all patterns of one table must have the same length")
        blob = "".join(patterns).encode("ascii")
        self._check(self.lib.tps_set_patterns(self._h, blob, len(patterns), k))
        self.patterns = list(patterns)

    def set_patterns_wide(self, patterns: list[str]):
        if not patterns:
            raise TopsicleHipError("empty pattern list")
        k = len(patterns[0])
        if any(len(p) != k for p in patterns):
            raise TopsicleHipError("all patterns of one table must have the same length")
        blob = "".join(patterns).encode("ascii", "replace")
        self._check(self.lib.tps_set_patterns_wide(self._h, blob, len(patterns), k))
        self.patterns = list(patterns)

    def upload(self, slot: int, bases: np.ndarray, offsets: np.ndarray):
        bases = np.ascontiguousarray(bases, dtype=np.uint8)
        offsets = np.ascontiguousarray(offsets, dtype=np.int64)
        n = len(offsets) - 1
        self._check(self.lib.tps_batch_upload(self._h, slot, _ptr(bases), _ptr(offsets), n))
        self._n[slot] = n

    def upload_packed(self, slot: int, seq2: np.ndarray, inv, desc: np.ndarray):
        assert seq2.dtype == np.uint32 and desc.dtype == DESC_DTYPE and (inv is None or inv.dtype == np.uint16)
        n, nw = len(desc), len(seq2)
        assert inv is None or len(inv) == nw
        self._check(self.lib.tps_batch_upload_packed(self._h, slot, _ptr(seq2), _ptr(inv), _ptr(desc), n, nw))
        self._n[slot] = n

    def upload_nib4(self, slot: int, nib: np.ndarray, src: np.ndarray, desc: np.ndarray, n_words: int):
        assert nib.dtype == np.uint8 and src.dtype == NIB_SRC_DTYPE and desc.dtype == DESC_DTYPE and len(src) == len(desc)
        n = len(desc)
# ... 260 lines not shown
```

Measured before the change: 4069 billion.

## Store fused-variant window sums as 8-bit per-tile slots instead of 16-bit

Adds an 8-bit window-sum storage mode for the fused variant path when the maximum window count fits in a byte (no self-overlap, no duplicates, no raw store). Each tile writes its sums into a fixed 512-byte slot using packed 64-bit buffer stores. Binseg reads through a view that indexes these slots, and the host widens them back to int32. This halves the global traffic for sum writes and reads. The cost is padded slot layout, extra index arithmetic in binseg, and a second layout path to maintain.

```diff
diff --git a/__graft_entry__.py b/__graft_entry__.py
--- a/__graft_entry__.py
+++ b/__graft_entry__.py
@@ -72,6 +72,7 @@
     import emu_follow_wide_driver
     import emu_motif_driver
     import emu_place_driver
+    import emu_sums8_driver
     import emu_tract_driver
     import emu_variant_driver
     import emu_wide_driver
@@ -97,6 +98,8 @@
     emu_clear_driver.build_main()
     import test_layout
     test_layout.build_main()
+    emu_sums8_driver.build()
+    emu_sums8_driver.build_main()
 
 
 def build_sanitizer_variants():
diff --git a/include/topsicle_hip.h b/include/topsicle_hip.h
--- a/include/topsicle_hip.h
+++ b/include/topsicle_hip.h
@@ -177,6 +177,7 @@
 int  tps_kernel_time_reset(tps_ctx* ctx);
 int  tps_ctx_debug_option(tps_ctx* ctx, const char* key, int64_t value);
 int  tps_debug_stamps_get(tps_ctx* ctx, int32_t slot, uint64_t* out, int64_t n_reads);
+int  tps_debug_sums_bits(tps_ctx* ctx, int32_t slot);
 int  tps_device_info(tps_ctx* ctx, char* buf, int32_t buf_len);
 int  tps_batch_kernel_info(tps_ctx* ctx, int32_t slot, char* buf, int32_t buf_len);
 
diff --git a/topsicle_amd/csrc/topsicle_hip.hip b/topsicle_amd/csrc/topsicle_hip.hip
--- a/topsicle_amd/csrc/topsicle_hip.hip
+++ b/topsicle_amd/csrc/topsicle_hip.hip
@@ -310,13 +310,14 @@
 };
 
 struct Slot {
-    DevBuf seq2, inv, desc, tails, results, c_start, c_end, win_off, win_off16, sums, raw, stamps, lc, order;
+    DevBuf seq2, inv, desc, tails, results, c_start, c_end, win_off, win_off16, base8, sums, raw, stamps, lc, order;
     int64_t n_words = 0;
     bool inv_valid = true;
     bool any_invalid = true;
     std::vector<int64_t> h_offsets;
     tps::BatchLayout lay;
     std::vector<uint16_t> h_sums16;
+    std::vector<uint8_t> h_sums8;
     tps_read_result* h_results = nullptr;
     size_t h_results_cap = 0;
     int64_t n = -1;
@@ -818,6 +819,7 @@
         sl.args = tps::ScanArgs{};
         sl.args.val_on = sl.any_invalid ? 1 : 0;
         if ((rc = plan_lds(c, sl, prm, sl.lay.max_nwin))) return rc;
+        if (inner) sl.args.sw8 = 0;
         sl.stride_base = 0;
         if (!inner && !c->no_stride) {
             sl.stride_base = tps::stride_base(sl.args, prm, c->pat.k, P, [&](int s0) { return window_count(sl.lay.max_len, prm.window, s0, prm.trimfirst, prm.maxlen); },
@@ -825,7 +827,11 @@
         }
         if ((rc = sl.win_off.ensure((size_t)(n + 1) * 8))) return rc;
         HIP_TRY(hipMemcpyAsync(sl.win_off.p, sl.lay.win_off.data(), (size_t)(n + 1) * 8, hipMemcpyHostToDevice, c->stream));
-        if (sl.args.variant) {
+        if (sl.args.variant && sl.args.sw8) {
+            tps::plan_sums8_layout(sl.lay, sl.args.tw);
+            if ((rc = sl.base8.ensure((size_t)(n + 1) * 8))) return rc;
+            HIP_TRY(hipMemcpyAsync(sl.base8.p, sl.lay.base8.data(), (size_t)(n + 1) * 8, hipMemcpyHostToDevice, c->stream));
+        } else if (sl.args.variant) {
             if ((rc = sl.win_off16.ensure((size_t)(n + 1) * 8))) return rc;
             HIP_TRY(hipMemcpyAsync(sl.win_off16.p, sl.lay.win_off16.data(), (size_t)(n + 1) * 8, hipMemcpyHostToDevice, c->stream));
         }
@@ -864,9 +870,15 @@
     a.sums = nullptr;
     a.sums16 = nullptr;
     a.win_off16 = nullptr;
+    a.sums8 = nullptr;
+    a.base8 = nullptr;
     a.raw = nullptr;
     if (prm.flags & TPS_F_WINDOWS) {
-        if (a.variant) {
+        if (a.variant && a.sw8) {
+            if ((rc = sl.sums.ensure((size_t)std::max<int64_t>(sl.lay.base8[(size_t)n], tps::SW8_SLOT)))) return rc;
+            a.sums8 = (uint8_t*)sl.sums.p;
+            a.base8 = (const int64_t*)sl.base8.p;
+        } else if (a.variant) {
             if ((rc = sl.sums.ensure((size_t)std::max<int64_t>(sl.lay.win_off16[(size_t)n], 8) * 2))) return rc;
             a.sums16 = (uint16_t*)sl.sums.p;
             a.win_off16 = (const int64_t*)sl.win_off16.p;
@@ -898,7 +910,7 @@
         if (inner) TPS_POISON(sl.results);
         else if ((rc = poison_h_results(c, sl))) return rc;
         if (a.c_start) { TPS_POISON(sl.c_start); TPS_POISON(sl.c_end); }
-        if (a.sums || a.sums16) TPS_POISON(sl.sums);
+        if (a.sums || a.sums16 || a.sums8) TPS_POISON(sl.sums);
         if (a.raw && !sl.rows_inline) TPS_POISON(sl.raw);
         if (a.lc_scratch) TPS_POISON(sl.lc);
     }
@@ -1719,7 +1731,12 @@
     if ((rc = need_scanned(c, slot, &sl))) return rc;
     if (!(sl->last_flags & TPS_F_STORE_SUMS)) return fail(TPS_E_STATE, "last scan did not store window sums");
     if (nw != sl->lay.win_off[(size_t)sl->n] || (nw > 0 && !sums)) return fail(TPS_E_ARG, "sums must hold %lld windows", (long long)sl->lay.win_off[(size_t)sl->n]);
-    if (nw && sl->args.variant) {
+    if (nw && sl->args.variant && sl->args.sw8) {
+        const int64_t n8 = sl->lay.base8[(size_t)sl->n];
+        sl->h_sums8.resize((size_t)n8);
+        HIP_TRY(hipMemcpy(sl->h_sums8.data(), sl->sums.p, (size_t)n8, hipMemcpyDeviceToHost));
+        tps::widen_sums8(sl->h_sums8.data(), sl->lay.base8.data(), sl->lay.win_off.data(), sl->lay.tw8, 0, sl->n, sums);
+    } else if (nw && sl->args.variant) {
         const int64_t n16 = sl->lay.win_off16[(size_t)sl->n];
         sl->h_sums16.resize((size_t)n16);
         HIP_TRY(hipMemcpy(sl->h_sums16.data(), sl->sums.p, (size_t)n16 * 2, hipMemcpyDeviceToHost));
@@ -1740,7 +1757,12 @@
     const int64_t lo = sl->lay.win_off[(size_t)read], cnt = sl->lay.win_off[(size_t)read + 1] - lo;
     if (nw != cnt || (nw > 0 && !sums)) return fail(TPS_E_ARG, "sums must hold %lld windows", (long long)cnt);
     if (!nw) return TPS_OK;
-    if (sl->args.variant) {
+    if (sl->args.variant && sl->args.sw8) {
+        const int64_t b0 = sl->lay.base8[(size_t)read], nb = sl->lay.base8[(size_t)read + 1] - b0;
+        sl->h_sums8.resize((size_t)nb);
+        HIP_TRY(hipMemcpy(sl->h_sums8.data(), (const uint8_t*)sl->sums.p + b0, (size_t)nb, hipMemcpyDeviceToHost));
+        tps::widen_sums8(sl->h_sums8.data(), sl->lay.base8.data(), sl->lay.win_off.data(), sl->lay.tw8, read, read + 1, sums);
+    } else if (sl->args.variant) {
         sl->h_sums16.resize((size_t)nw);
         HIP_TRY(hipMemcpy(sl->h_sums16.data(), (const uint16_t*)sl->sums.p + sl->lay.win_off16[(size_t)read], (size_t)nw * 2, hipMemcpyDeviceToHost));
         for (int64_t w = 0; w < nw; ++w) sums[w] = (int32_t)sl->h_sums16[(size_t)w];
@@ -2012,6 +2034,14 @@
     return TPS_OK;
 }
 
+int tps_debug_sums_bits(tps_ctx* c, int32_t slot) {
+    Slot* sl;
+    int rc;
+    if ((rc = need_scanned(c, slot, &sl))) return rc;
+    const Slot* s = (sl->stride_base && sl->sub) ? sl->sub : sl;
+    return !s->args.variant ? 32 : s->args.sw8 ? 8 : 16;
+}
+
 int tps_debug_stamps_get(tps_ctx* c, int32_t slot, uint64_t* out, int64_t n) {
     Slot* sl;
     int rc;
diff --git a/topsicle_amd/csrc/tps_device.h b/topsicle_amd/csrc/tps_device.h
--- a/topsicle_amd/csrc/tps_device.h
+++ b/topsicle_amd/csrc/tps_device.h
@@ -84,6 +84,9 @@
     int32_t xt_alias;
     int32_t xt_own;
     int32_t pair16;
+    int32_t sw8;
+    uint8_t* sums8;
+    const int64_t* base8;
 };
 
 struct BinsegArgs {
@@ -916,12 +919,21 @@
     uint32_t jump, jump_magic, lc_cap;
     uint64_t lc_g;
     uint16_t* sw16;
+    int32_t sw8;
     int64_t rd;
 };
+template <bool LC>
 TPS_DEV TileConst tile_const(const ScanArgs& a, int64_t r) {
     TileConst t;
     t.lc_g = (uint64_t)(uintptr_t)(a.lc_scratch + r * (int64_t)a.lc_stride);
     t.sw16 = a.sums16 + (a.win_off16 ? a.win_off16[r] : 0);
+    t.sw8 = 0;
+    if constexpr (LC) {
+        if (a.sums8) {
+            t.sw16 = (uint16_t*)(a.sums8 + a.base8[r]);
+            t.sw8 = 1;
+        }
+    }
     t.rd = r;
     t.q = (int32_t)uniform((uint32_t)a.q); t.r = (int32_t)uniform((uint32_t)a.r);
     t.jump = uniform((uint32_t)a.prm.jump); t.jump_magic = uniform(a.jump_magic);
@@ -1692,7 +1704,12 @@
     TPS_PHASE {
         const int lane = tid;
         const uint32_t* const sw = TPS_AT(sw_);
-        if constexpr (SWP) g_store_sw8p(tc.sw16 + w0, lane, nw_tile, TPS_AT(swp_));
+        if (CD == 0 && tc.sw8) {
+            uint8_t* const slot = (uint8_t*)tc.sw16 + tile * SW8_SLOT;
+            if constexpr (SWP) g_store_sw8bp(slot, lane, nw_tile, TPS_AT(swp_));
+            else g_store_sw8b(slot, lane, nw_tile, sw);
+        }
+        else if constexpr (SWP) g_store_sw8p(tc.sw16 + w0, lane, nw_tile, TPS_AT(swp_));
         else g_store_sw8(tc.sw16 + w0, lane, nw_tile, sw);
         uint32_t* pr = l.row + lane * (B + 1);
         uint32_t run = 0;
@@ -2247,8 +2264,16 @@
     int need = ((min_size + jump - 1) / jump) * jump + min_size;
     return need <= n;
 }
+struct SwView {
+    const uint8_t* p;
+    int tw;
+    TPS_DEVM uint32_t operator[](int w) const {
+        if (tw) return p[(w / tw) * SW8_SLOT + w % tw];
+        return ((const uint16_t*)p)[w];
+    }
+};
 template <typename ST>
-TPS_DEV Cand binseg_chunk(const ST* S, int n, int jump, int min_size, int lo, int hi, uint64_t prefix, uint64_t total) {
+TPS_DEV Cand binseg_chunk(ST S, int n, int jump, int min_size, int lo, int hi, uint64_t prefix, uint64_t total) {
     Cand best{0, 1, -1};
     uint64_t run = prefix;
     for (int b = lo; b < hi; ++b) {
@@ -2271,7 +2296,7 @@
 }
 
 template <typename ST>
-TPS_DEV Cand binseg_exact_wg(const ST* S, int n, int jump, int min_size, uint32_t* xs) {
+TPS_DEV Cand binseg_exact_wg(ST S, int n, int jump, int min_size, uint32_t* xs) {
     const int cl = (n + NT - 1) / NT;
     TPS_PHASE {
         int lo = tid * cl, hi = lo + cl < n ? lo + cl : n;
@@ -2409,7 +2434,7 @@
 }
 
 template <typename ST>
-TPS_DEV void binseg_from_lc(const ScanArgs& a, const Lds& l, uint64_t lc_g, const ST* S_global, int n, uint64_t tot, int jump,
+TPS_DEV void binseg_from_lc(const ScanArgs& a, const Lds& l, uint64_t lc_g, ST S_global, int n, uint64_t tot, int jump,
                             int min_size, int n_patterns, uint32_t* misc, uint32_t* xs, int& bkp, double& gain, bool& tie) {
     const int ncand = (n - 1) / jump;
     Lane<double> best_(-1.0);
@@ -2783,7 +2808,7 @@
         } else {
             typedef TileGeo<SV ? SV : 1, FULL> t_;
             constexpr int PF = t_::PF;
-            const TileConst tc = tile_const(a, r);
+            const TileConst tc = tile_const<!SO && !RAW>(a, r);
             int tw = (int)uniform((uint32_t)a.tw);
             TPS_PIN_S(tw);
             bool pp = false;
@@ -2963,7 +2988,10 @@
         bool tie = false;
         TPS_FENCE_WG();
         const uint64_t lc_g = a.lc_global ? (uint64_t)(uintptr_t)(a.lc_scratch + r * (int64_t)a.lc_stride) : 0ull;
-        if constexpr (SV != 0)
+        if constexpr (SV != 0 && !SO && !RAW) {
+            const SwView sv{a.sums8 ? (const uint8_t*)(a.sums8 + a.base8[r]) : (const uint8_t*)(a.sums16 + (a.win_off16 ? a.win_off16[r] : 0)), a.sums8 ? a.tw : 0};
+            binseg_from_lc(a, l, lc_g, sv, n_win, s_total, prm.jump, prm.min_size, pat.P, l.misc, l.blk, bkp, gain, tie);
+        } else if constexpr (SV != 0)
             binseg_from_lc(a, l, lc_g, (const uint16_t*)(a.sums16 + (a.win_off16 ? a.win_off16[r] : 0)), n_win, s_total, prm.jump, prm.min_size, pat.P,
                            l.misc, l.blk, bkp, gain, tie);
         else
diff --git a/topsicle_amd/csrc/tps_plan.h b/topsicle_amd/csrc/tps_plan.h
--- a/topsicle_amd/csrc/tps_plan.h
+++ b/topsicle_amd/csrc/tps_plan.h
@@ -38,10 +38,13 @@
 }
 
 inline int64_t sums16_slots(int64_t nw) { return (nw + 7) & ~7ll; }
+inline int64_t sums8_bytes(int64_t nw, int tw) { return tw > 0 ? ((nw + tw - 1) / tw) * (int64_t)SW8_SLOT : 0; }
 
 struct BatchLayout {
     std::vector<int64_t> win_off;
     std::vector<int64_t> win_off16;
+    std::vector<int64_t> base8;
+    int32_t tw8 = 0;
     std::vector<int32_t> order;
     int64_t max_nwin = 0;
     int64_t max_len = 0;
@@ -50,6 +53,8 @@
     lay.win_off.resize((size_t)n + 1);
     lay.win_off16.resize((size_t)n + 1);
     lay.max_nwin = lay.max_len = 0;
+    lay.base8.clear();
+    lay.tw8 = 0;
     std::vector<int64_t> nwv((size_t)n);
     std::vector<uint8_t> longer((size_t)n);
     int64_t acc = 0, acc16 = 0;
@@ -68,6 +73,25 @@
     lay.win_off[(size_t)n] = acc;
     lay.win_off16[(size_t)n] = acc16;
     plan_dispatch_order(nwv.data(), longer.data(), n, lay.order);
+}
+
+inline void plan_sums8_layout(BatchLayout& lay, int tw) {
+    const size_t n = lay.win_off.empty() ? 0 : lay.win_off.size() - 1;
+    lay.base8.assign(n + 1, 0);
+    lay.tw8 = tw;
+    for (size_t i = 0; i < n; ++i) lay.base8[i + 1] = lay.base8[i] + sums8_bytes(lay.win_off[i + 1] - lay.win_off[i], tw);
+}
+
+inline void widen_sums8(const uint8_t* src8, const int64_t* base8, const int64_t* win_off, int tw, int64_t r0, int64_t r1, int32_t* dst) {
+    for (int64_t i = r0; i < r1; ++i) {
+        const uint8_t* s = src8 + (base8[i] - base8[r0]);
+        int32_t* d = dst + (win_off[i] - win_off[r0]);
+        const int64_t cnt = win_off[i + 1] - win_off[i];
+        for (int64_t w0 = 0; w0 < cnt; w0 += tw, s += SW8_SLOT) {
+            const int64_t m = std::min<int64_t>(tw, cnt - w0);
+            for (int64_t w = 0; w < m; ++w) d[w0 + w] = (int32_t)s[w];
+        }
+    }
 }
 
 inline void widen_sums16(const uint16_t* src16, const int64_t* win_off16, const int64_t* win_off, int64_t r0, int64_t r1, int32_t* dst) {
@@ -271,7 +295,7 @@
                        a.q / 8 + 2 < (XLANES - NT) && max_period <= std::min(prm.slide, 6) &&
                        2 * a.head_dw <= fused_seq_dw(prm.slide);
     a.tw = 0; a.pair_n = 0; a.lc_global = 0; a.lc_stride = 0; a.pp_d = -1; a.so_fast = 0; a.seq_alias = 0; a.lut_fields = 0; a.tile_full = 0;
-    a.lut16 = 0; a.xt_alias = 0; a.xt_own = 0; a.pair16 = 0;
+    a.lut16 = 0; a.xt_alias = 0; a.xt_own = 0; a.pair16 = 0; a.sw8 = 0;
     if (fused) {
         const bool pp_counts = a.pat.dup_mask == 0 && k >= 4 && P <= 14 && (8 * prm.slide + k - 1) / k <= 14 && (prm.slide + k - 1) / k <= 2 &&
                                a.lw / k + 2 <= 127;
@@ -306,6 +330,7 @@
         if (a.pat.so_mask == 0 && !(prm.flags & TPS_F_STORE_RAW)) a.seq_alias = 1;
 #endif
         a.tw = ((int)NT * 8 - a.q - 1) & ~1;
+        a.sw8 = (a.pat.so_mask == 0 && a.pat.dup_mask == 0 && !(prm.flags & TPS_F_STORE_RAW) && a.lw + P <= 255) ? 1 : 0;
         a.lc_global = 1;
         a.lc_stride = 2 * ((a.lc_cap + 1) & ~1);
         a.pair_n = (a.pat.so_mask == 0 && k <= 4 && !(prm.flags & TPS_F_STORE_RAW)) ? (1 << (2 * (k + 1))) : 0;
@@ -335,7 +360,7 @@
         }
         if (wg_lds_dwords(a) <= budget_dw) return "";
         a.tw = 0; a.pair_n = 0; a.lc_global = 0; a.lc_stride = 0; a.pp_d = -1; a.so_fast = 0; a.seq_alias = 0; a.lut_fields = 0;
-        a.lut16 = 0; a.xt_alias = 0; a.xt_own = 0; a.pair16 = 0;
+        a.lut16 = 0; a.xt_alias = 0; a.xt_own = 0; a.pair16 = 0; a.sw8 = 0;
     }
     a.variant = 0;
     a.lc_global = 1;
diff --git a/topsicle_amd/csrc/tps_wave.h b/topsicle_amd/csrc/tps_wave.h
--- a/topsicle_amd/csrc/tps_wave.h
+++ b/topsicle_amd/csrc/tps_wave.h
@@ -3,6 +3,7 @@
 
 #ifdef TPS_EMU
 #define TPS_DEV static inline
+#define TPS_DEVM inline
 #define TPS_HD static inline
 #define TPS_AT(x) ((x).v[tid])
 #define TPS_PHASE for (int tid = 0; tid < tps::NT; ++tid)
@@ -16,6 +17,7 @@
 #define TPS_PIN_V(x) ((void)0)
 #else
 #define TPS_DEV __device__ __forceinline__
+#define TPS_DEVM __device__ __forceinline__
 #define TPS_HD __host__ __device__ inline
 #define TPS_AT(x) (x)
 __device__ __forceinline__ int tps_fresh_lane() {
@@ -389,6 +391,36 @@
     __builtin_amdgcn_raw_buffer_store_b128(t, rs, lane * 16, 0, STORE_AUX);
 }
 #endif
+constexpr int SW8_SLOT = 512;
+#ifdef TPS_EMU
+TPS_DEV void g_store_sw8b(uint8_t* slot_out, int lane, int nw_tile, const uint32_t* v) {
+    const int end = (nw_tile + 3) & ~3;
+    for (int i = 0; i < 8; ++i)
+        if (8 * lane + (i & ~3) < end) slot_out[8 * lane + i] = (uint8_t)v[i];
+}
+TPS_DEV void g_store_sw8bp(uint8_t* slot_out, int lane, int nw_tile, const uint32_t* p) {
+    const int end = (nw_tile + 3) & ~3;
+    for (int i = 0; i < 8; ++i)
+        if (8 * lane + (i & ~3) < end) slot_out[8 * lane + i] = (uint8_t)(p[i >> 1] >> (16 * (i & 1)));
+}
+#else
+TPS_DEV void g_store_sw8b(uint8_t* slot_out, int lane, int nw_tile, const uint32_t* v) {
+    typedef unsigned int v2u __attribute__((ext_vector_type(2)));
+    const __amdgpu_buffer_rsrc_t rs = __builtin_amdgcn_make_buffer_rsrc((void*)slot_out, 0, (nw_tile + 3) & ~3, 0x00020000);
+    v2u t;
+    t.x = v[0] | (v[1] << 8) | (v[2] << 16) | (v[3] << 24);
+    t.y = v[4] | (v[5] << 8) | (v[6] << 16) | (v[7] << 24);
+    __builtin_amdgcn_raw_buffer_store_b64(t, rs, lane * 8, 0, STORE_AUX);
+}
+TPS_DEV void g_store_sw8bp(uint8_t* slot_out, int lane, int nw_tile, const uint32_t* p) {
+    typedef unsigned int v2u __attribute__((ext_vector_type(2)));
+    const __amdgpu_buffer_rsrc_t rs = __builtin_amdgcn_make_buffer_rsrc((void*)slot_out, 0, (nw_tile + 3) & ~3, 0x00020000);
+    v2u t;
+    t.x = perm(p[1], p[0], 0x06040200u);
+    t.y = perm(p[3], p[2], 0x06040200u);
+    __builtin_amdgcn_raw_buffer_store_b64(t, rs, lane * 8, 0, STORE_AUX);
+}
+#endif
 #ifdef TPS_EMU
 TPS_DEV void g_store16_clamped(uint32_t* base, int n_dw, int cdw, const u32x4& t) {
     const uint32_t v[4] = {t.x, t.y, t.z, t.w};
diff --git a/topsicle_amd/hiplib.py b/topsicle_amd/hiplib.py
--- a/topsicle_amd/hiplib.py
+++ b/topsicle_amd/hiplib.py
@@ -19,7 +19,7 @@
     "tps_batch_download_packed", "tps_batch_kmer_followers", "tps_batch_kmer_followers_wide", "tps_batch_motif_census", "tps_batch_variant_census", "tps_batch_tract_map", "tps_batch_end_sketch", "tps_sketch_links", "tps_batch_end_window", "tps_window_offsets", "tps_window_place", "tps_batch_adapter_find", "tps_batch_set_tails", "tps_batch_scan", "tps_sync",
     "tps_batch_results", "tps_batch_window_offsets", "tps_batch_window_sums", "tps_batch_window_raw",
     "tps_batch_raw_to_fd", "tps_batch_trc_counts", "tps_trc_counts", "tps_window_counts", "tps_binseg_l2", "tps_binseg_l2_ties", "tps_batch_read_sums", "tps_window_count",
-    "tps_kernel_time_ms", "tps_kernel_time_reset", "tps_device_info", "tps_batch_kernel_info", "tps_ctx_debug_option", "tps_debug_stamps_get",
+    "tps_kernel_time_ms", "tps_kernel_time_reset", "tps_device_info", "tps_batch_kernel_info", "tps_ctx_debug_option", "tps_debug_stamps_get", "tps_debug_sums_bits",
 ]
 
 
@@ -130,6 +130,7 @@
         "tps_batch_kernel_info": (C.c_int, [vp, i32, C.c_char_p, i32]),
         "tps_ctx_debug_option": (C.c_int, [vp, C.c_char_p, i64]),
         "tps_debug_stamps_get": (C.c_int, [vp, i32, vp, i64]),
+        "tps_debug_sums_bits": (C.c_int, [vp, i32]),
     }
     for name, (res, args) in proto.items():
         try:
@@ -267,6 +268,12 @@
         self._check(self.lib.tps_debug_stamps_get(self._h, slot, _ptr(out), n))
         return out
 
+    def sums_bits(self, slot: int) -> int:
+        bits = self.lib.tps_debug_sums_bits(self._h, slot)
+        if bits < 0:
+            self._check(bits)
+        return bits
+
     def helper(self, j: int) -> "HipScanner":
         while len(self._helpers) <= j:
             h = HipScanner(self.device, self._lib_path)
```

Result: faster. 4154 billion (median of 5 runs) (+2.1%).
